# sleepybishop/nanorq

Measured on AMD Instinct MI355X. Metric: Gbit/s encode+decode, K=8192 T=1280, higher is better.
Workload: dtype u8

## Files before the change

__graft_entry__.py:

```python
import os
import sys

ROOT = os.path.dirname(os.path.abspath(__file__))
for p in (ROOT, os.path.join(ROOT, "tests")):
    if p not in sys.path:
        sys.path.insert(0, p)


def build():
    from nanorq_amd import build as nbuild
    nbuild.build_lib(verbose=True)
    nbuild.build_emu()
    nbuild.build_planner_emu()
    nbuild.build_ingest_emu()
    nbuild.build_emit_emu()
    nbuild.build_held_emu()
    nbuild.build_rxset_emu()
    nbuild.build_rxset_lists_emu()
    nbuild.build_rxset_want_emu()
    nbuild.build_txset_emu()
    nbuild.build_syms_emu()
    nbuild.build_syms_set_emu()
    nbuild.build_runs_emu()
    nbuild.build_rxset_runs_emu()
    nbuild.build_obj_emu()
    nbuild.build_shape_emu()
    nbuild.build_launch_emu()
    nbuild.build_out_lists_emu()
    nbuild.build_model_lib()
    nbuild.build_rows_probe()
    nbuild.build_tools()
    import oracle
    oracle.build()
    if os.path.isfile("/root/reference/benchmark.c"):
        import subprocess
        subprocess.run(["make", "-s", "-C", os.path.join(ROOT, "oracle"), "_ref/benchmark_hip", "_ref/encode_hip", "_ref/decode_hip"],
                       check=True)
    import nanorq_amd
    nanorq_amd.lib()
    print("build ok:", nanorq_amd.lib_path())


def smoke():
    import numpy as np
    import nanorq_amd
    import oracle
    import gpu_support as G
    from util import payload, loss_pattern

    K, T, nblk = 1024, 1280, 2
    src = np.stack([payload(K * T, seed=1, block=b).reshape(K, T) for b in range(nblk)])
    lost = [loss_pattern(K, 0.05, seed=2, block=b) for b in range(nblk)]
    nrep = max(len(l) for l in lost) + 2
    esis = np.arange(K, K + nrep, dtype=np.uint32)
    rep, inter = G.gpu_encode(src, K, T, esis, want_inter=True)
    for b in range(nblk):
        r_rep, r_int, _ = oracle.encode_block(src[b], K, T, esis, want_inter=True)
        assert np.array_equal(inter[b], r_int), "intermediate symbols differ from the oracle"
        assert np.array_equal(rep[b], r_rep), "repair symbols differ from the oracle"
    work = src.copy()
    for b in range(nblk):
        work[b][lost[b]] = 0
    st, out, _ = G.gpu_decode(work, K, T, lost, [esis[:len(l) + 2] for l in lost],
                              [rep[b][:len(lost[b]) + 2] for b in range(nblk)])
    assert st.all() and np.array_equal(out, src), "decode mismatch"
    print("smoke ok: K=%d T=%d blocks=%d, stats=%s" % (K, T, nblk, G.ctx().stats()))


if __name__ == "__main__":
    build()
    if "--smoke" in sys.argv:
        smoke()
```

include/nanorq_hip.h:

```cpp
#ifndef NANORQ_HIP_H
#define NANORQ_HIP_H

#include <stddef.h>
#include <stdint.h>

#ifdef __cplusplus
extern "C" {
#endif

typedef struct nrq_ctx nrq_ctx;

typedef struct nrq_call_stats {
  double plan_ms;
  double host_ms;
  uint32_t strip_bytes;
  uint32_t lds_bytes;
  uint32_t grid;
  uint32_t planner;
  uint64_t plan_bytes;
  uint64_t xor_ops;
  uint32_t npiv, u, nlev, nfree;
  uint32_t wg_threads;
  uint32_t strips_per_slot;
  uint32_t wg_waves_per_simd;
  uint32_t host_planned;
  uint32_t movers_aligned;
  uint32_t plan_ahead;
  uint32_t strip_bytes_b, blocks_b;
  uint32_t plan_wg_threads;
  uint32_t plan_compact_state;
  uint32_t plan_segmented;
  uint32_t backsub_strip;
  uint32_t encplan_device;
} nrq_call_stats;

int nrq_ctx_create(int device, void *stream, nrq_ctx **out);
void nrq_ctx_destroy(nrq_ctx *ctx);
int nrq_ctx_set_stream(nrq_ctx *ctx, void *stream);
const char *nrq_ctx_error(nrq_ctx *ctx);
int nrq_ctx_sync(nrq_ctx *ctx);
void nrq_ctx_last_stats(nrq_ctx *ctx, nrq_call_stats *out);
int nrq_ctx_set_planner(nrq_ctx *ctx, int device_planner);
int nrq_ctx_set_option(nrq_ctx *ctx, const char *name, long long value);
int nrq_ctx_set_threads(nrq_ctx *ctx, int n);

int nrq_params(uint32_t K, uint32_t out[10]);

int nrq_precalculate(nrq_ctx *ctx, uint32_t K, uint32_t Kp);
int nrq_warm(nrq_ctx *ctx, uint32_t K, uint32_t Kp, int encode_plan);
void nrq_plan_cache_clear(nrq_ctx *ctx);

int nrq_encode_blocks(nrq_ctx *ctx, uint32_t K, uint32_t Kp, uint32_t T, uint32_t nblk, const void *d_src, size_t src_stride,
                      void *d_inter, size_t inter_stride, uint32_t nrep, const uint32_t *h_esis, void *d_rep,
                      size_t rep_stride);

int nrq_decode_blocks(nrq_ctx *ctx, uint32_t K, uint32_t Kp, uint32_t T, uint32_t nblk, void *d_src, size_t src_stride,
                      const uint32_t *h_lost, const uint32_t *h_nlost, uint32_t lost_cap, const uint32_t *h_rep_esi,
                      const uint32_t *h_nrep, uint32_t rep_cap, const void *d_rep, size_t rep_stride, void *d_inter,
                      size_t inter_stride, int *h_status);

int nrq_decode_blocks_lazy(nrq_ctx *ctx, uint32_t K, uint32_t Kp, uint32_t T, uint32_t nblk, void *d_src, size_t src_stride,
                           const uint32_t *h_lost, const uint32_t *h_nlost, uint32_t lost_cap, const uint32_t *h_rep_esi,
                           const uint32_t *h_nrep, const uint32_t *h_nrep_avail, uint32_t rep_cap, const void *d_rep,
                           size_t rep_stride, void *d_inter, size_t inter_stride, int *h_status, uint32_t *h_used);

int nrq_decode_plan_ahead(nrq_ctx *ctx, uint32_t K, uint32_t Kp, uint32_t T, uint32_t nblk, void *d_src, size_t src_stride,
                          const uint32_t *h_lost, const uint32_t *h_nlost, uint32_t lost_cap, const uint32_t *h_rep_esi,
                          const uint32_t *h_nrep, const uint32_t *h_nrep_avail, uint32_t rep_cap, const void *d_rep, size_t rep_stride,
                          void *d_inter, size_t inter_stride);

int nrq_encode_blocks_v(nrq_ctx *ctx, uint32_t K, uint32_t Kp, uint32_t T, uint32_t nblk, const void *d_src, size_t src_stride,
                        const uint64_t *d_inter_v);
int nrq_decode_blocks_v(nrq_ctx *ctx, uint32_t K, uint32_t Kp, uint32_t T, uint32_t nblk, const uint64_t *d_src_v, const uint32_t *h_lost,
                        const uint32_t *h_nlost, uint32_t lost_cap, const uint32_t *h_rep_esi, const uint32_t *h_nrep,
                        const uint32_t *h_nrep_avail, uint32_t rep_cap, const uint64_t *d_rep_v, int *h_status, uint32_t *h_used);

int nrq_decode_blocks_vi(nrq_ctx *ctx, uint32_t K, uint32_t Kp, uint32_t T, uint32_t nblk, const uint64_t *d_src_v, const uint32_t *h_lost,
                         const uint32_t *h_nlost, uint32_t lost_cap, const uint32_t *h_rep_esi, const uint32_t *h_nrep,
                         const uint32_t *h_nrep_avail, uint32_t rep_cap, const uint64_t *d_rep_v, const uint64_t *d_inter_v, int *h_status,
                         uint32_t *h_used);

int nrq_decode_blocks_vc(nrq_ctx *ctx, uint32_t K, uint32_t Kp, uint32_t T, uint32_t nblk, const uint64_t *d_src_v, const uint32_t *h_lost,
                         const uint32_t *h_nlost, uint32_t lost_cap, const uint32_t *h_rep_esi, const uint32_t *h_nrep,
                         const uint32_t *h_nrep_avail, uint32_t rep_cap, const uint64_t *d_rep_v, int *h_status, uint32_t *h_used,
                         uint32_t chunk_blocks, void *const *chunk_done, void *const *upload_done);

int nrq_gen_symbols(nrq_ctx *ctx, uint32_t K, uint32_t Kp, uint32_t T, uint32_t nblk, const void *d_inter, size_t inter_stride,
                    uint32_t n, const uint32_t *h_isi, void *d_out, size_t out_stride);

int nrq_gen_symbols_dev(nrq_ctx *ctx, uint32_t K, uint32_t Kp, uint32_t T, uint32_t nblk, const void *d_inter, size_t inter_stride,
                        uint32_t n, const uint32_t *d_isi, void *d_out, size_t out_stride);

int nrq_dev_alloc(nrq_ctx *ctx, size_t bytes, void **out);
int nrq_dev_free(nrq_ctx *ctx, void *p);
int nrq_dev_upload(nrq_ctx *ctx, void *d_dst, const void *h_src, size_t bytes);
int nrq_dev_download(nrq_ctx *ctx, void *h_dst, const void *d_src, size_t bytes);
int nrq_dev_memset(nrq_ctx *ctx, void *d_dst, int value, size_t bytes);
int nrq_dev_upload_async(nrq_ctx *ctx, void *d_dst, const void *h_src, size_t bytes);
int nrq_dev_download_async(nrq_ctx *ctx, void *h_dst, const void *d_src, size_t bytes);
int nrq_dev_copy(nrq_ctx *ctx, void *d_dst, const void *d_src, size_t bytes);

int nrq_dev_trim(nrq_ctx *ctx);
int nrq_dev_pool_books(nrq_ctx *ctx, size_t out[3]);

int nrq_host_alloc_pinned(size_t bytes, void **out);
void nrq_host_free_pinned(void *p);
int nrq_host_register(void *p, size_t bytes);
void nrq_host_unregister(void *p);
int nrq_host_is_pinned(const void *p);
int nrq_host_range_is_pinned(const void *p, size_t bytes);
int nrq_copy_on(nrq_ctx *ctx, int stream, void *dst, const void *src, size_t bytes);
int nrq_memset_on(nrq_ctx *ctx, int stream, void *d_dst, int value, size_t bytes);
int nrq_event_new(nrq_ctx *ctx, void **out);
void nrq_event_free(void *ev);
int nrq_event_record(nrq_ctx *ctx, void *ev, int stream);
int nrq_stream_wait(nrq_ctx *ctx, int stream, void *ev);
// ... 154 lines not shown
```

nanorq_amd/binding.py:

```python
import ctypes as C
import os

import numpy as np

_HERE = os.path.dirname(os.path.abspath(__file__))
_LIB = None


class NrqError(RuntimeError):
    pass


class ObjParams(C.Structure):
    _fields_ = [("F", C.c_uint64)] + [(n, C.c_uint32) for n in
                                       ("T", "Al", "Z", "N", "Kt", "ZL", "KL", "KpL", "ZS", "KS", "KpS", "NL", "TL", "NS", "TS",
                                        "flags", "max_esi")] + [("oti_common", C.c_uint64), ("oti_specific", C.c_uint32)]

    def as_dict(self):
        return {n: getattr(self, n) for n, _ in self._fields_}


class CallStats(C.Structure):
    _fields_ = [("plan_ms", C.c_double), ("host_ms", C.c_double), ("strip_bytes", C.c_uint32),
                ("lds_bytes", C.c_uint32), ("grid", C.c_uint32), ("planner", C.c_uint32),
                ("plan_bytes", C.c_uint64), ("xor_ops", C.c_uint64), ("npiv", C.c_uint32), ("u", C.c_uint32),
                ("nlev", C.c_uint32), ("nfree", C.c_uint32), ("wg_threads", C.c_uint32), ("strips_per_slot", C.c_uint32),
                ("wg_waves_per_simd", C.c_uint32), ("host_planned", C.c_uint32), ("movers_aligned", C.c_uint32),
                ("plan_ahead", C.c_uint32), ("strip_bytes_b", C.c_uint32), ("blocks_b", C.c_uint32),
                ("plan_wg_threads", C.c_uint32), ("plan_compact_state", C.c_uint32), ("plan_segmented", C.c_uint32),
                ("backsub_strip", C.c_uint32), ("encplan_device", C.c_uint32)]

    def as_dict(self):
        return {k: getattr(self, k) for k, _ in self._fields_}


def lib_path():
    return os.path.join(_HERE, "libnanorq_hip.so")


def lib():
    global _LIB
    if _LIB is not None:
        return _LIB
    from . import build
    path = os.environ.get("NANORQ_HIP_LIB") or build.build_lib()
    L = C.CDLL(path)
    vp, u32p, ip = C.c_void_p, C.POINTER(C.c_uint32), C.POINTER(C.c_int)
    sz = C.c_size_t
    L.nrq_ctx_create.argtypes = [C.c_int, vp, C.POINTER(vp)]
    L.nrq_ctx_destroy.argtypes = [vp]
    L.nrq_ctx_destroy.restype = None
    L.nrq_ctx_set_stream.argtypes = [vp, vp]
    L.nrq_ctx_error.argtypes = [vp]
    L.nrq_ctx_error.restype = C.c_char_p
    L.nrq_ctx_sync.argtypes = [vp]
    L.nrq_ctx_last_stats.argtypes = [vp, C.POINTER(CallStats)]
    L.nrq_ctx_last_stats.restype = None
    L.nrq_ctx_set_threads.argtypes = [vp, C.c_int]
    L.nrq_ctx_set_planner.argtypes = [vp, C.c_int]
    L.nrq_ctx_set_option.argtypes = [vp, C.c_char_p, C.c_longlong]
    L.nrq_params.argtypes = [C.c_uint32, u32p]
    L.nrq_precalculate.argtypes = [vp, C.c_uint32, C.c_uint32]
    L.nrq_plan_cache_clear.argtypes = [vp]
    L.nrq_plan_cache_clear.restype = None
    L.nrq_encode_blocks.argtypes = [vp, C.c_uint32, C.c_uint32, C.c_uint32, C.c_uint32, vp, sz, vp, sz, C.c_uint32, u32p, vp, sz]
    L.nrq_decode_blocks.argtypes = [vp, C.c_uint32, C.c_uint32, C.c_uint32, C.c_uint32, vp, sz, u32p, u32p, C.c_uint32, u32p,
                                    u32p, C.c_uint32, vp, sz, vp, sz, ip]
    L.nrq_decode_blocks_lazy.argtypes = [vp, C.c_uint32, C.c_uint32, C.c_uint32, C.c_uint32, vp, sz, u32p, u32p, C.c_uint32,
                                         u32p, u32p, u32p, C.c_uint32, vp, sz, vp, sz, ip, u32p]
    L.nrq_decode_plan_ahead.argtypes = [vp, C.c_uint32, C.c_uint32, C.c_uint32, C.c_uint32, vp, sz, u32p, u32p, C.c_uint32,
                                        u32p, u32p, u32p, C.c_uint32, vp, sz, vp, sz]
    L.nrq_gen_symbols.argtypes = [vp, C.c_uint32, C.c_uint32, C.c_uint32, C.c_uint32, vp, sz, C.c_uint32, u32p, vp, sz]
    L.nrq_dev_alloc.argtypes = [vp, sz, C.POINTER(vp)]
    L.nrq_dev_free.argtypes = [vp, vp]
    if hasattr(L, "nrq_dev_pool_books"):
        L.nrq_dev_pool_books.argtypes = [vp, C.POINTER(sz)]
    L.nrq_dev_trim.argtypes = [vp]
    L.nrq_dev_upload.argtypes = [vp, vp, vp, sz]
    L.nrq_dev_download.argtypes = [vp, vp, vp, sz]
    L.nrq_dev_memset.argtypes = [vp, vp, C.c_int, sz]
    L.nrq_ktime_enable.argtypes = [vp, C.c_int]
    L.nrq_ktime_read.argtypes = [vp, C.POINTER(C.c_float), C.c_uint32, u32p]
    L.nrq_ptime_read.argtypes = [vp, C.POINTER(C.c_float), C.c_uint32, u32p]
    L.nrq_ktime_read_intervals.argtypes = [vp, vp, C.POINTER(C.c_float), C.POINTER(C.c_float), C.c_uint32, u32p]
    L.nrq_timer_start.argtypes = [vp]
    L.nrq_timer_stop_ms.argtypes = [vp, C.POINTER(C.c_float)]
    L.nrq_rx_create.argtypes = [vp, C.c_uint32, C.c_uint32, C.c_uint32, C.c_uint32, C.c_uint32, C.c_uint32, C.c_uint32, vp, sz, vp, sz,
                                C.POINTER(vp)]
    L.nrq_rx_destroy.argtypes = [vp]
    L.nrq_rx_destroy.restype = None
    L.nrq_rx_add.argtypes = [vp, vp, sz, vp, C.c_uint32, C.c_uint32, vp]
    L.nrq_rx_counts.argtypes = [vp, u32p, u32p]
    L.nrq_rx_lists.argtypes = [vp, u32p, u32p, u32p, u32p]
    L.nrq_rx_decode.argtypes = [vp, ip, u32p]
    L.nrq_rx_src.argtypes = [vp]
    L.nrq_rx_src.restype = vp
    L.nrq_rx_rep.argtypes = [vp]
    L.nrq_rx_rep.restype = vp
    L.nrq_rx_reset.argtypes = [vp]
    L.nrq_tx_create.argtypes = [vp, C.c_uint32, C.c_uint32, C.c_uint32, C.c_uint32, C.c_uint32, vp, sz, C.POINTER(vp)]
    L.nrq_tx_destroy.argtypes = [vp]
    L.nrq_tx_destroy.restype = None
    L.nrq_tx_encode.argtypes = [vp]
    L.nrq_tx_emit.argtypes = [vp, vp, C.c_uint32, vp, sz, C.c_uint32, vp]
    L.nrq_tx_emit_range.argtypes = [vp, C.c_uint32, C.c_uint32, C.c_int, vp, sz, C.c_uint32, vp]
    L.nrq_tx_inter.argtypes = [vp]
    L.nrq_tx_inter.restype = vp
    opp = C.POINTER(ObjParams)
    L.nrq_obj_params_enc.argtypes = [C.c_uint64, C.c_uint32, C.c_uint32, C.c_uint32, C.c_uint32, C.c_uint32, C.c_uint32, opp]
    L.nrq_obj_params_oti.argtypes = [C.c_uint64, C.c_uint32, C.c_uint32, opp]
    L.nrq_obj_layout.argtypes = [vp, opp, vp, vp, C.c_int]
    L.nrq_otx_create.argtypes = [vp, opp, vp, C.POINTER(vp)]
    L.nrq_otx_destroy.argtypes = [vp]
# ... 3 lines not shown
    L.nrq_otx_emit_all.argtypes = [vp, C.c_uint32, C.c_int, vp, sz, C.c_uint32, vp]
    L.nrq_otx_oti.argtypes = [vp, C.POINTER(C.c_uint64), u32p]
    L.nrq_orx_create.argtypes = [vp, opp, C.c_uint32, C.POINTER(vp)]
    L.nrq_orx_destroy.argtypes = [vp]
    L.nrq_orx_destroy.restype = None
    L.nrq_orx_add.argtypes = [vp, vp, sz, vp, C.c_uint32, C.c_uint32, vp]
    L.nrq_orx_counts.argtypes = [vp, u32p, u32p]
    L.nrq_orx_decode.argtypes = [vp, ip, u32p]
    L.nrq_orx_write.argtypes = [vp, vp]
    if hasattr(L, "nrq_rx_relay"):
        L.nrq_tx_ready.argtypes = [vp, u32p]
        L.nrq_rx_relay.argtypes = [vp, C.POINTER(vp)]
        L.nrq_otx_ready.argtypes = [vp, u32p]
        L.nrq_orx_relay.argtypes = [vp, C.POINTER(vp)]
    if hasattr(L, "nrq_rx_held"):
        L.nrq_rx_held.argtypes = [vp, vp, C.c_uint32, u32p]
        L.nrq_orx_held.argtypes = [vp, vp, C.c_uint32, u32p]
    if hasattr(L, "nrq_rx_want"):
        L.nrq_rx_want.argtypes = [vp, C.c_uint32, C.c_uint32, C.c_uint32, vp, C.c_uint32, u32p]
        L.nrq_orx_want.argtypes = [vp, C.c_uint32, C.c_uint32, C.c_uint32, vp, C.c_uint32, u32p]
    if hasattr(L, "nrq_rxset_create"):
        L.nrq_rxset_create.argtypes = [vp, C.c_uint32, C.POINTER(vp)]
        L.nrq_rxset_destroy.argtypes = [vp]
        L.nrq_rxset_destroy.restype = None
        L.nrq_rxset_attach.argtypes = [vp, C.c_uint32, vp]
        L.nrq_rxset_attach_obj.argtypes = [vp, C.c_uint32, vp]
        L.nrq_rxset_detach.argtypes = [vp, C.c_uint32]
        L.nrq_rxset_add.argtypes = [vp, vp, sz, vp, vp, C.c_uint32, C.c_uint32, vp]
    if hasattr(L, "nrq_rxset_decode"):
        L.nrq_rxset_blocks.argtypes = [vp, u32p, u32p, C.c_uint32, u32p]
        L.nrq_rxset_counts.argtypes = [vp, u32p, u32p]
        L.nrq_rxset_lists.argtypes = [vp, u32p, u32p, u32p, sz, C.POINTER(sz)]
        L.nrq_rxset_decode.argtypes = [vp, ip, u32p]
    if hasattr(L, "nrq_rxset_want"):
        L.nrq_rxset_want.argtypes = [vp, C.c_uint32, C.c_uint32, C.c_uint32, vp, vp, C.c_uint32, u32p, u32p]
        L.nrq_rxset_held.argtypes = [vp, vp, vp, C.c_uint32, u32p, u32p]
    if hasattr(L, "nrq_txset_create"):
        L.nrq_txset_create.argtypes = [vp, C.c_uint32, C.POINTER(vp)]
        L.nrq_txset_destroy.argtypes = [vp]
        L.nrq_txset_destroy.restype = None
        L.nrq_txset_attach.argtypes = [vp, C.c_uint32, vp]
        L.nrq_txset_attach_obj.argtypes = [vp, C.c_uint32, vp]
        L.nrq_txset_detach.argtypes = [vp, C.c_uint32]
        L.nrq_txset_blocks.argtypes = [vp, u32p, u32p, C.c_uint32, u32p]
        L.nrq_txset_emit.argtypes = [vp, vp, vp, C.c_uint32, vp, sz, C.c_uint32, vp]
    if hasattr(L, "nrq_rx_add_syms"):
        u32 = C.c_uint32
        L.nrq_pkt_count.argtypes = [u32, u32, u32, u32]
        L.nrq_pkt_count.restype = u32
        L.nrq_rx_add_syms.argtypes = [vp, vp, sz, vp, u32, u32, vp, u32, vp]
        L.nrq_orx_add_syms.argtypes = [vp, vp, sz, vp, u32, u32, vp, u32, vp]
        L.nrq_tx_emit_syms.argtypes = [vp, vp, u32, u32, vp, vp, sz, u32, vp]
        L.nrq_otx_emit_syms.argtypes = [vp, vp, u32, u32, vp, vp, sz, u32, vp]
        L.nrq_tx_emit_range_syms.argtypes = [vp, u32, u32, u32, C.c_int, vp, sz, u32, vp, vp, u32p]
        L.nrq_otx_emit_all_syms.argtypes = [vp, u32, u32, C.c_int, vp, sz, u32, vp, vp, u32p]
    if hasattr(L, "nrq_rxset_add_syms"):
        u32 = C.c_uint32
        L.nrq_rxset_add_syms.argtypes = [vp, vp, sz, vp, vp, u32, u32, vp, u32, vp]
        L.nrq_txset_emit_syms.argtypes = [vp, vp, vp, u32, u32, vp, vp, sz, u32, vp]
    if hasattr(L, "nrq_rx_want_syms"):
        u32 = C.c_uint32
        L.nrq_rx_want_syms.argtypes = [vp, u32, u32, u32, u32, vp, vp, u32, u32p, u32p]
        L.nrq_orx_want_syms.argtypes = [vp, u32, u32, u32, u32, vp, vp, u32, u32p, u32p]
        L.nrq_rx_held_syms.argtypes = [vp, u32, vp, vp, u32, u32p, u32p]
        L.nrq_orx_held_syms.argtypes = [vp, u32, vp, vp, u32, u32p, u32p]
    if hasattr(L, "nrq_rxset_want_syms"):
        u32 = C.c_uint32
        L.nrq_rxset_want_syms.argtypes = [vp, u32, u32, u32, u32, vp, vp, vp, u32, u32p, u32p, u32p]
        L.nrq_rxset_held_syms.argtypes = [vp, u32, vp, vp, vp, u32, u32p, u32p, u32p]
    u8pp = C.POINTER(C.POINTER(C.c_uint8))
    L.nrq_host_kconst_build.argtypes = [C.c_uint32, u8pp, u32p]
    L.nrq_host_plan_build.argtypes = [C.c_uint32, C.c_uint32, u32p, C.POINTER(C.c_uint8), u8pp, u32p]
    L.nrq_host_plan_build_forced.argtypes = [C.c_uint32, C.c_uint32, u32p, C.POINTER(C.c_uint8), u8pp, u32p, C.c_uint32]
    L.nrq_host_free.argtypes = [vp]
    L.nrq_host_free.restype = None
    _LIB = L
    return L


PARAM_NAMES = ("Kp", "J", "S", "H", "W", "L", "P", "P1", "U", "B")
PLAN_FIELDS = ("magic status K Kp J S H W L P P1 B M npiv u nlow r2 nfree nlev nrows pipe wpr "
               "npiv_pad n_xor_ops off_ops off_pivslot off_pivcol off_wt off_lowslot off_pivx off_fbits "
               "off_mh off_freex off_hinv off_colslot off_pivof off_uslot total_bytes reserved0 reserved1 fail_site "
               "off_augt lpr aug_stride nneed need_pad off_needslot off_wneed").split()


def params(K):
    out = (C.c_uint32 * 10)()
    if lib().nrq_params(K, out) != 0:
        raise ValueError("K out of range: %r" % (K,))
    return dict(zip(PARAM_NAMES, (int(x) for x in out)))


def _u32(a):
    return a.ctypes.data_as(C.POINTER(C.c_uint32))


def host_kconst(K):
    out = C.POINTER(C.c_uint8)()
    n = C.c_uint32()
    if lib().nrq_host_kconst_build(K, C.byref(out), C.byref(n)) != 0:
        raise NrqError("kconst build failed")
    buf = bytes(C.string_at(out, n.value))
    lib().nrq_host_free(out)
    return buf


def host_plan(K, isis, kconst, extra_inact=0):
    isis = np.ascontiguousarray(isis, dtype=np.uint32)
    kc = (C.c_uint8 * len(kconst)).from_buffer_copy(kconst)
    out = C.POINTER(C.c_uint8)()
    n = C.c_uint32()
    rc = lib().nrq_host_plan_build_forced(K, len(isis), _u32(isis), kc, C.byref(out), C.byref(n), int(extra_inact))
    if rc != 0:
        raise NrqError("plan build failed: %d" % rc)
    buf = bytes(C.string_at(out, n.value))
    lib().nrq_host_free(out)
    return buf


def plan_header(plan):
    h = np.frombuffer(plan, dtype=np.uint32, count=len(PLAN_FIELDS))
    return dict(zip(PLAN_FIELDS, (int(x) for x in h)))


class Context:

    def __init__(self, device=0, stream=None):
        self._L = lib()
        h = C.c_void_p()
        rc = self._L.nrq_ctx_create(device, C.c_void_p(stream or 0), C.byref(h))
        if rc != 0:
            raise NrqError("nrq_ctx_create failed (%d): no usable HIP device -- the HIP path has no CPU fallback" % rc)
        self._h = h
        self.device = device

    def close(self):
        if getattr(self, "_h", None):
            self._L.nrq_ctx_destroy(self._h)
            self._h = None

    def __del__(self):
        try:
            self.close()
        except Exception:
            pass

    def _chk(self, rc):
        if rc != 0:
            raise NrqError("%s (rc=%d)" % (self._L.nrq_ctx_error(self._h).decode(), rc))

    def set_stream(self, stream):
        self._chk(self._L.nrq_ctx_set_stream(self._h, C.c_void_p(stream or 0)))

    def set_planner(self, device=True):
        self._chk(self._L.nrq_ctx_set_planner(self._h, int(bool(device))))

    def set_option(self, name, value):
        self._chk(self._L.nrq_ctx_set_option(self._h, name.encode(), int(value)))

    def set_threads(self, n):
        self._chk(self._L.nrq_ctx_set_threads(self._h, n))

    def sync(self):
        self._chk(self._L.nrq_ctx_sync(self._h))

    def stats(self):
# ... 777 lines not shown
```

nanorq_amd/build.py:

```python
import os
import shutil
import subprocess
import sys

HERE = os.path.dirname(os.path.abspath(__file__))
ROOT = os.path.dirname(HERE)
CSRC = os.path.join(HERE, "csrc")
LIB = os.path.join(HERE, "libnanorq_hip.so")
EMU = os.path.join(ROOT, "tests", "emu", "libsolve_emu.so")
PEMU = os.path.join(ROOT, "tests", "emu", "libplanner_emu.so")
IEMU = os.path.join(ROOT, "tests", "emu", "libingest_emu.so")
XEMU = os.path.join(ROOT, "tests", "emu", "libemit_emu.so")
OEMU = os.path.join(ROOT, "tests", "emu", "libobj_emu.so")
SEMU = os.path.join(ROOT, "tests", "emu", "libshape_emu.so")
HEMU = os.path.join(ROOT, "tests", "emu", "libheld_emu.so")
WEMU = os.path.join(ROOT, "tests", "emu", "libwant_emu.so")
REMU = os.path.join(ROOT, "tests", "emu", "librxset_emu.so")
LEMU = os.path.join(ROOT, "tests", "emu", "librxset_lists_emu.so")
QEMU = os.path.join(ROOT, "tests", "emu", "librxset_want_emu.so")
TEMU = os.path.join(ROOT, "tests", "emu", "libtxset_emu.so")
YEMU = os.path.join(ROOT, "tests", "emu", "libsyms_emu.so")
ZEMU = os.path.join(ROOT, "tests", "emu", "libsyms_set_emu.so")
GEMU = os.path.join(ROOT, "tests", "emu", "libruns_emu.so")
JEMU = os.path.join(ROOT, "tests", "emu", "librxset_runs_emu.so")
NEMU = os.path.join(ROOT, "tests", "emu", "liblaunch_emu.so")
UEMU = os.path.join(ROOT, "tests", "emu", "libout_lists_emu.so")
MODEL = os.path.join(ROOT, "tests", "emu", "libnanorq_model.so")
ROWS = os.path.join(ROOT, "tests", "gpu", "librows_probe.so")

HIP_SOURCES = ["nrq_device.hip"]
CXX_SOURCES = ["planner_host.cpp"]
C_SOURCES = ["nanorq_api.c", "io.c"]


def _hipcc():
    for c in (os.environ.get("HIPCC"), "/opt/rocm/bin/hipcc", shutil.which("hipcc")):
        if c and os.path.exists(c):
            return c
    raise RuntimeError("hipcc not found: the HIP extension cannot be built (no CPU fallback exists)")


def _newer(target, deps):
    if not os.path.exists(target):
        return True
    t = os.path.getmtime(target)
    return any(os.path.getmtime(d) > t for d in deps if os.path.exists(d))


def _deps():
    out = []
    for d in (CSRC, os.path.join(ROOT, "include")):
        for f in os.listdir(d):
            out.append(os.path.join(d, f))
    return out


def build_lib(force=False, verbose=False, out=None, extra=(), host_extra=(), reuse_hip_obj=False):
    if out is None and not force and not _newer(LIB, _deps()):
        return LIB
    hipcc = _hipcc()
    objdir = os.path.join(HERE, "build" if out is None else "build_" + os.path.basename(out))
    os.makedirs(objdir, exist_ok=True)
    objs = []
    common = ["-O3", "-fPIC", "-Wno-pass-failed", "-I" + os.path.join(ROOT, "include"), "-I" + CSRC]
    common += list(extra)
    headers = [f for f in _deps() if f.endswith(".h")]

    def stale(o, src):
        return force or out is not None or _newer(o, [src] + headers)

    for s in HIP_SOURCES:
        o = os.path.join(objdir, s + ".o")
        if reuse_hip_obj and os.path.exists(os.path.join(HERE, "build", s + ".o")):
            objs.append(os.path.join(HERE, "build", s + ".o"))
            continue
        if stale(o, os.path.join(CSRC, s)):
            subprocess.run([hipcc, "--offload-arch=gfx950", "-std=c++17", *common, "-c", os.path.join(CSRC, s), "-o", o],
                           check=True)
        objs.append(o)
    for s in CXX_SOURCES:
        o = os.path.join(objdir, s + ".o")
        if stale(o, os.path.join(CSRC, s)):
            subprocess.run(["g++", "-std=c++17", "-Wall", *common, *host_extra, "-c", os.path.join(CSRC, s), "-o", o], check=True)
        objs.append(o)
    for s in C_SOURCES:
        src = os.path.join(CSRC, s)
        if not os.path.exists(src):
            continue
        o = os.path.join(objdir, s + ".o")
        if stale(o, src):
            subprocess.run(["gcc", "-std=gnu11", "-Wall", "-D_FILE_OFFSET_BITS=64", *common, *host_extra, "-c", src, "-o", o], check=True)
        objs.append(o)
    target = out or LIB
    subprocess.run([hipcc, "--offload-arch=gfx950", "-shared", "-fPIC", "-o", target, *objs, "-lpthread"], check=True)
    if verbose:
        print("built", target)
    return target


def build_tools(force=False):
    src = os.path.join(ROOT, "tools", "rqfile.c")
    exe = os.path.join(ROOT, "tools", "rqfile")
    deps = [src, LIB] + [os.path.join(ROOT, "include", h) for h in ("nanorq.h", "nanorq_batch.h", "io.h")]
    if force or _newer(exe, deps):
        subprocess.run(["gcc", "-std=c99", "-D_DEFAULT_SOURCE", "-D_FILE_OFFSET_BITS=64", "-O2", "-Wall", "-I" + os.path.join(ROOT, "include"),
                        src, "-o", exe, "-L" + os.path.dirname(LIB), "-lnanorq_hip", "-Wl,-rpath,$ORIGIN/../nanorq_amd", "-lm"], check=True)
    return exe


def _build_emu(target, src, headers, force):
    if force or _newer(target, [src] + [os.path.join(CSRC, h) for h in headers]):
        subprocess.run(["g++", "-O2", "-std=c++17", "-Wall", "-Wno-unknown-pragmas", "-fPIC", "-shared", "-o", target, src], check=True)
    return target


def build_emu(force=False):
    return _build_emu(EMU, os.path.join(ROOT, "tests", "emu", "solve_emu.cpp"),
                      ("solve_body.h", "split_body.h", "plan.h", "rq_math.h", os.path.join(ROOT, "tests", "emu", "strip_emu.h")), force)


def build_launch_emu(force=False):
    return _build_emu(NEMU, os.path.join(ROOT, "tests", "emu", "launch_emu.cpp"),
                      ("launch_shape.h", "planner_body.h", "solve_body.h", "split_body.h", "plan.h", "rq_math.h", "rfc6330_tables.h",
                       os.path.join(ROOT, "tests", "emu", "strip_emu.h"), os.path.join(ROOT, "tests", "emu", "wave_emu.h")), force)


def build_planner_emu(force=False):
    return _build_emu(PEMU, os.path.join(ROOT, "tests", "emu", "planner_emu.cpp"),
                      ("planner_body.h", "planner_seq.h", "solve_body.h", "plan.h", "rq_math.h"), force)


def build_out_lists_emu(force=False):
    return _build_emu(UEMU, os.path.join(ROOT, "tests", "emu", "out_lists_emu.cpp"), ("out_lists.h", "rq_math.h"), force)


def build_ingest_emu(force=False):
    return _build_emu(IEMU, os.path.join(ROOT, "tests", "emu", "ingest_emu.cpp"), ("ingest_body.h",), force)


def build_emit_emu(force=False):
    return _build_emu(XEMU, os.path.join(CSRC, "emit_emu.cpp"), ("emit_emu.h", "emit_body.h", "rq_math.h"), force)


def build_held_emu(force=False):
    return _build_emu(HEMU, os.path.join(CSRC, "held_emu.cpp"), ("emit_emu.h", "emit_body.h", "held_body.h", "ingest_body.h", "rq_math.h"), force)


def build_want_emu(force=False):
    return _build_emu(WEMU, os.path.join(CSRC, "want_emu.cpp"), ("want_body.h", "held_body.h", "ingest_body.h"), force)


def build_rxset_emu(force=False):
    return _build_emu(REMU, os.path.join(CSRC, "rxset_emu.cpp"), ("ingest_set_body.h", "ingest_body.h"), force)


def build_rxset_lists_emu(force=False):
    return _build_emu(LEMU, os.path.join(CSRC, "rxset_lists_emu.cpp"),
                      ("lists_set_body.h", "rxset_plan.h", "ingest_set_body.h", "ingest_body.h"), force)


def build_rxset_want_emu(force=False):
    return _build_emu(QEMU, os.path.join(CSRC, "rxset_want_emu.cpp"),
                      ("emu_scan.h", "want_set_body.h", "lists_set_body.h", "want_body.h", "held_body.h", "ingest_set_body.h", "ingest_body.h"), force)


def build_txset_emu(force=False):
    return _build_emu(TEMU, os.path.join(CSRC, "txset_emu.cpp"), ("emit_set_body.h", "emit_body.h", "rq_math.h"), force)


def build_syms_emu(force=False):
    return _build_emu(YEMU, os.path.join(CSRC, "syms_emu.cpp"), ("emit_emu.h", "syms_body.h", "emit_body.h", "ingest_body.h", "rq_math.h"), force)


def build_syms_set_emu(force=False):
    return _build_emu(ZEMU, os.path.join(CSRC, "syms_set_emu.cpp"),
                      ("syms_set_body.h", "syms_body.h", "ingest_set_body.h", "emit_set_body.h", "emit_body.h", "ingest_body.h", "rq_math.h"), force)


def build_runs_emu(force=False):
    return _build_emu(GEMU, os.path.join(CSRC, "runs_emu.cpp"),
                      ("emit_emu.h", "runs_emu_walks.h", "runs_body.h", "syms_body.h", "want_body.h", "held_body.h", "emit_body.h", "ingest_body.h",
                       "rq_math.h"), force)


def build_rxset_runs_emu(force=False):
    return _build_emu(JEMU, os.path.join(CSRC, "rxset_runs_emu.cpp"),
                      ("emu_scan.h", "runs_emu_walks.h", "runs_set_body.h", "runs_body.h", "syms_set_body.h", "want_set_body.h", "lists_set_body.h",
                       "syms_body.h", "want_body.h", "held_body.h", "emit_set_body.h", "emit_body.h", "ingest_set_body.h", "ingest_body.h", "rq_math.h"), force)


def build_obj_emu(force=False):
    return _build_emu(OEMU, os.path.join(ROOT, "tests", "emu", "obj_emu.cpp"), ("obj_body.h", "emit_body.h", "rq_math.h"), force)


def build_shape_emu(force=False):
    return _build_emu(SEMU, os.path.join(ROOT, "tests", "emu", "shape_emu.cpp"),
                      ("launch_shape.h", "planner_body.h", "solve_body.h", "plan.h", "rq_math.h", "rfc6330_tables.h"), force)


def build_model_lib(force=False, out=None, sanitize=False):
    emu = os.path.join(ROOT, "tests", "emu")
    hook, model, effects = os.path.join(emu, "hip_model.h"), os.path.join(emu, "hip_model.cpp"), os.path.join(emu, "model_effects.cpp")
    target = out or MODEL
    if not force and not _newer(target, _deps() + [hook, model, effects]):
        return target
    hipcc = _hipcc()
    rocm = os.path.dirname(os.path.dirname(os.path.realpath(hipcc)))
    objdir = os.path.join(HERE, "build_model" if out is None else "build_" + os.path.basename(out))
    os.makedirs(objdir, exist_ok=True)
    common = ["-O2", "-g1", "-fPIC", "-I" + os.path.join(ROOT, "include"), "-I" + CSRC, "-I" + emu]
    cc, cxx, san, hip_san = "gcc", "g++", [], []
    if sanitize:
        llvm = os.path.join(rocm, "lib", "llvm", "bin")
        cc, cxx = os.path.join(llvm, "clang"), os.path.join(llvm, "clang++")
        san = ["-O1", "-fno-omit-frame-pointer", "-fsanitize=address,undefined", "-fno-sanitize-recover=undefined"]
        hip_san = [x for f in san for x in ("-Xarch_host", f)]
    objs = []

    def obj(cmd, src, name):
        o = os.path.join(objdir, name + ".o")
        subprocess.run([*cmd, *common, "-c", src, "-o", o], check=True)
        objs.append(o)
        return o

    dev = obj([hipcc, "--offload-host-only", "-std=c++17", "-Wno-pass-failed", "-DNRQ_HIP_MODEL_HOOK", "-include", hook, *hip_san],
              os.path.join(CSRC, HIP_SOURCES[0]), HIP_SOURCES[0])
    for s in CXX_SOURCES:
        obj([cxx, "-std=c++17", "-Wall", *san], os.path.join(CSRC, s), s)
    for s in C_SOURCES:
        obj([cc, "-std=gnu11", "-Wall", "-D_FILE_OFFSET_BITS=64", *san], os.path.join(CSRC, s), s)
    obj([cxx, "-std=c++17", "-Wall", "-D__HIP_PLATFORM_AMD__", "-I" + os.path.join(rocm, "include"), *san], model, "hip_model.cpp")
    obj([cxx, "-std=c++17", "-Wall", "-Wno-unknown-pragmas", *[f for f in san if f != "-fsanitize=address,undefined"],
         *(["-fsanitize=undefined"] if sanitize else [])], effects, "model_effects.cpp")
    undefined = subprocess.run(["nm", "-u", dev], check=True, stdout=subprocess.PIPE).stdout.decode().split()
    defs = ["-Wl,--defsym=%s=0" % n for n in undefined if n.startswith("__hip_fatbin")]
    subprocess.run([cxx, "-shared", "-fPIC", *san, "-o", target, *objs, *defs, "-lpthread", "-ldl"], check=True)
    return target


def build_rows_probe(force=False):
    src = os.path.join(ROOT, "tests", "gpu", "rows_probe.hip")
    if force or _newer(ROWS, [src, os.path.join(CSRC, "solve_body.h"), os.path.join(CSRC, "plan.h")]):
        subprocess.run([_hipcc(), "--offload-arch=gfx950", "-O3", "-std=c++17", "-I" + CSRC, "-shared", "-fPIC", src, "-o", ROWS], check=True)
    return ROWS


def build_model_exercise(force=False, sanitize=True):
    emu = os.path.join(ROOT, "tests", "emu")
    src = os.path.join(emu, "model_exercise.cpp")
    exe = os.path.join(emu, "model_exercise_asan" if sanitize else "model_exercise")
    lib = build_model_lib(force=force, out=os.path.join(emu, "libnanorq_model_asan.so") if sanitize else None, sanitize=sanitize)
    if force or _newer(exe, [src, lib]):
        cxx, san = "g++", []
        if sanitize:
            cxx = os.path.join(os.path.dirname(os.path.dirname(os.path.realpath(_hipcc()))), "lib", "llvm", "bin", "clang++")
            san = ["-O1", "-fno-omit-frame-pointer", "-fsanitize=address,undefined", "-fno-sanitize-recover=undefined"]
        subprocess.run([cxx, "-std=c++17", "-Wall", "-g1", *san, "-I" + os.path.join(ROOT, "include"), "-I" + emu, src, "-o", exe,
                        "-L" + emu, "-l:" + os.path.basename(lib), "-Wl,-rpath,$ORIGIN", "-lpthread"], check=True)
    return exe


if __name__ == "__main__":
    build_lib(force="-f" in sys.argv, verbose=True)
    build_emu(force="-f" in sys.argv)
    build_planner_emu(force="-f" in sys.argv)
    build_ingest_emu(force="-f" in sys.argv)
    build_emit_emu(force="-f" in sys.argv)
    build_held_emu(force="-f" in sys.argv)
    build_want_emu(force="-f" in sys.argv)
    build_rxset_emu(force="-f" in sys.argv)
    build_rxset_lists_emu(force="-f" in sys.argv)
    build_rxset_want_emu(force="-f" in sys.argv)
    build_txset_emu(force="-f" in sys.argv)
    build_syms_emu(force="-f" in sys.argv)
    build_syms_set_emu(force="-f" in sys.argv)
    build_runs_emu(force="-f" in sys.argv)
    build_rxset_runs_emu(force="-f" in sys.argv)
    build_obj_emu(force="-f" in sys.argv)
    build_shape_emu(force="-f" in sys.argv)
    build_launch_emu(force="-f" in sys.argv)
    build_out_lists_emu(force="-f" in sys.argv)
    build_model_lib(force="-f" in sys.argv)
    build_rows_probe(force="-f" in sys.argv)
    build_tools(force="-f" in sys.argv)
```

nanorq_amd/csrc/nrq_device.hip:

```cpp
#include <hip/hip_runtime.h>

#include <algorithm>
#include <atomic>
#include <chrono>
#include <cstdarg>
#include <cstdio>
#include <cstdlib>
#include <cstring>
#include <deque>
#include <map>
#include <new>
#include <string>
#include <thread>
#include <vector>

#include "../../include/nanorq_hip.h"
#include "plan.h"
#include "planner_host.h"
#include "rq_math.h"
#include "out_lists.h"
#include "solve_body.h"
#include "split_body.h"
#include "planner_body.h"
#include "ingest_body.h"
// ... 351 lines not shown
  pl_tag_pl_scan_b = 0,
  pl_tag_pl_scan_c = 0,
  pl_tag_pl_pcsc_fill = 0,
#endif
  pl_tag_pl_round_claim = 1,
  pl_tag_pl_round_drop = 3,
  pl_tag_pl_round_chain_end = 3,
  pl_tag_pl_inact_find = 5,
  pl_tag_pl_inact_find_b = 5,
  pl_tag_pl_inact_find_c = 5,
  pl_tag_pl_inact_apply_a = 6,
  pl_tag_pl_inact_apply_b = 6,
  pl_tag_pl_inact_next = 6,
  pl_tag_pl_event_scan = 5,
  pl_tag_pl_event_pick = 6,
  pl_tag_pl_event_drop = 6,
  pl_tag_pl_lev_0 = 7,
  pl_tag_pl_pivot_sort = 7,
  pl_tag_pl_lev_a = 7,
  pl_tag_pl_check_a = 7,
  pl_tag_pl_check_b = 7,
  pl_tag_pl_check_c = 7,
  pl_tag_pl_lev_b = 7,
  pl_tag_pl_w_init = 8,
  pl_tag_pl_w_init_b = 8,
  pl_tag_pl_cls_fetch = 8,
  pl_tag_pl_w_group = 8,
  pl_tag_pl_w_stage = 8,
  pl_tag_pl_wfast_spill = 4,
  pl_tag_pl_wfast_load = 4,
  pl_tag_pl_wfast_store = 4,
  pl_tag_pl_wfast_restore = 4,
  pl_tag_pl_low_a = 9,
  pl_tag_pl_low_b = 9,
  pl_tag_pl_low_c = 9,
  pl_tag_pl_ops_layout_a = 10,
  pl_tag_pl_ops_layout = 10,
  pl_tag_pl_ops_clear = 10,
  pl_tag_pl_ops_emit = 10,
  pl_tag_pl_ops_check_a = 10,
  pl_tag_pl_ops_check_b = 10,
  pl_tag_pl_ops_check_c = 10,
  pl_tag_pl_sh_restore = 0,
  pl_tag_pl_sh_save = 15,
  pl_tag_pl_mh_ext_clear = 15,
  pl_tag_pl_mh_fetch = 11,
  pl_tag_pl_mh_init = 11,
  pl_tag_pl_mh_load = 11,
  pl_tag_pl_mh_acc = 11,
  pl_tag_pl_gj_a = 12,
  pl_tag_pl_gjp_init = 12,
  pl_tag_pl_gjp_bid = 12,
  pl_tag_pl_gjp_step = 12,
  pl_tag_pl_gjp_wave = 12,
  pl_tag_pl_mhrev_load = 11,
  pl_tag_pl_mhrev_load_b = 11,
  pl_tag_pl_mhrev_store = 11,
  pl_tag_pl_mhrev_scatter = 11,
  pl_tag_pl_gjp_comb = 12,
  pl_tag_pl_gjp_stage = 12,
  pl_tag_pl_gjp_apply = 12,
  pl_tag_pl_gj_b = 12,
  pl_tag_pl_bin_a = 13,
  pl_tag_pl_bin_b = 13,
  pl_tag_pl_bin_c = 13,
  pl_tag_pl_dense_a = 14,
  pl_tag_pl_dense_b = 14,
  pl_tag_pl_dense_step_a = 14,
  pl_tag_pl_dense_step_b = 14,
  pl_tag_pl_dense_c = 14,
  pl_tag_pl_extra_a = 14,
  pl_tag_pl_extra_b = 14,
  pl_tag_pl_extra_c = 14,
  pl_tag_pl_extra_d = 14,
  pl_tag_pl_final_a = 15,
  pl_tag_pl_final_b = 15,
  pl_tag_pl_final_c = 15,
  pl_tag_pl_final_c2 = 15,
  pl_tag_pl_final_c3 = 15,
  pl_tag_pl_final_d = 15,
  pl_tag_pl_final_e = 15,
  pl_tag_pl_need_a = 15,
  pl_tag_pl_need_b = 15,
  pl_tag_pl_mark_failed = 15,
};

template <int NT, int PK = 0>
__global__ __launch_bounds__(NT) __attribute__((amdgpu_waves_per_eu(NT <= 256 ? 5 : 1)))
void nrq_plan_kernel(rq_params p, const uint8_t *__restrict__ kc,
                                                         const nrq_planjob *__restrict__ pjobs,
                                                         nrq_job *__restrict__ jobs_out, uint32_t nblk, uint32_t Mcap,
                                                         uint32_t npcap, uint32_t ucap, uint32_t lds_dyn_bytes,
                                                         unsigned long long *__restrict__ prof, uint32_t seg, uint32_t qcap,
                                                         uint32_t lowcap) {
  extern __shared__ __attribute__((aligned(16))) uint8_t smem[];
  const uint32_t b = blockIdx.x, tid = threadIdx.x;
#define PL_SEG_ (PK == 0 ? 0u : seg)
  if (b >= nblk) return;
  uint8_t *dyn = smem;
  pl_shared *sh = reinterpret_cast<pl_shared *>(smem + lds_dyn_bytes);
  PlanCtx c;
  pl_ctx_setup(c, p, kc, pjobs[b], sh, dyn, lds_dyn_bytes, Mcap, npcap, ucap, jobs_out + b, qcap, lowcap, (uint32_t)NT);
  if (!PK) c.pk_cnt = c.pk_un = c.pk_pa = c.pk_vb = nullptr;
  if (PL_SEG_ == 3u) c.cls_glob = reinterpret_cast<uint32_t *>(c.work + c.wl.cls_g);
  unsigned long long t_prev = prof ? (unsigned long long)clock64() : 0ull;
#ifdef PL_STAMP
#define PL_ACC(tag) ((void)0)
#else
#define PL_ACC(tag) do { if (__builtin_expect(prof && b == 0 && tid == 0, 0)) { unsigned long long t_ = (unsigned long long)clock64(); \
                                                          prof[tag] += t_ - t_prev; prof[16 + tag] += 1; t_prev = t_; } } while (0)
#endif
#define PL_PHASE(fn) do { fn<PK>(c, tid, (uint32_t)NT); __syncthreads(); PL_ACC(pl_tag_##fn); } while (0)
#define PL_PHASE1(fn, a) do { fn<PK>(c, (a), tid, (uint32_t)NT); __syncthreads(); PL_ACC(pl_tag_##fn); } while (0)
#ifndef PL_CLAIM_FULL_BARRIER
#define PL_CLAIM_FULL_BARRIER 0
#endif
#ifndef PL_CLAIM_SKIP_IDLE
#define PL_CLAIM_SKIP_IDLE 1
#endif
#define PL_PHASE1_CLAIM(fn, a) do { if (!PL_CLAIM_SKIP_IDLE || (tid & ~63u) < nq_) fn<PK>(c, (a), tid, (uint32_t)NT); \
    if (!PL_CLAIM_FULL_BARRIER && (pl_peel_in_lds(c) || c.pk_cnt)) asm volatile("s_waitcnt lgkmcnt(0)\n\ts_barrier" ::: "memory"); else __syncthreads(); \
    PL_ACC(pl_tag_##fn); } while (0)
#define PL_WFAST_RUN(wb) do { \
    if (tid < NRQ_ROW) { \
      const NRQ_GAS uint32_t *ops_ = gptr<uint32_t>(c.arena + c.sh->off_ops); \
      if ((wb) == 16u) fwd_rows<16>(ops_, pl_wfast_rows(c), tid); \
      else if ((wb) == 8u) fwd_rows<8>(ops_, pl_wfast_rows(c), tid); \
      else fwd_rows<4>(ops_, pl_wfast_rows(c), tid); \
    } \
    __syncthreads(); PL_ACC(2); } while (0)
#define PL_MHREV_RUN(wb) do { \
    if (tid < NRQ_ROW) { \
      const NRQ_GAS uint32_t *ops_ = gptr<uint32_t>(c.arena + c.sh->off_ops); \
      if ((wb) == 16u) rev_rows<16>(ops_, pl_wfast_rows(c), tid); \
      else if ((wb) == 8u) rev_rows<8>(ops_, pl_wfast_rows(c), tid); \
      else rev_rows<4>(ops_, pl_wfast_rows(c), tid); \
    } \
    __syncthreads(); PL_ACC(11); } while (0)
#define PL_SEG PL_SEG_
#define PL_STEER_SYNC __syncthreads()
#define PL_NT_ ((uint32_t)NT)
#define PL_Z ((uint32_t)PK)
#ifdef PL_STAMP
  c.st_on = prof && b == 0 && tid == 0; c.st_prev = 0; c.st_blk = prof && b == 0;
  if (tid < 32) sh->st_acc[tid] = 0;
  __syncthreads();
#endif
  if (PL_SEG_ == 2u || PL_SEG_ == 4u) PL_PHASE(pl_sh_restore);
#include "planner_seq.h"
#ifdef PL_STAMP
  if (c.st_on) { for (int i_ = 0; i_ < 32; i_++) prof[32 + i_] = sh->st_acc[i_]; }
#endif
  if (PL_SEG_ == 1u || PL_SEG_ == 4u) PL_PHASE(pl_mh_ext_clear);
  if (PL_SEG_ == 1u || PL_SEG_ == 3u || PL_SEG_ == 4u) PL_PHASE(pl_sh_save);
#undef PL_SEG
#undef PL_SEG_
#undef PL_STEER_SYNC
#undef PL_NT_
#undef PL_PHASE
#undef PL_PHASE1
#undef PL_PHASE1_CLAIM
#undef PL_WFAST_RUN
#undef PL_MHREV_RUN
#undef PL_Z
#undef PL_ACC
}
// ... 904 lines not shown
  if (rc) return rc;
  memset(&ctx->stats, 0, sizeof(ctx->stats));
  ctx->stats.plan_ms = cached ? 0.0 : ep->build_ms;
  ctx->stats.plan_bytes = ep->plan_bytes;
  ctx->stats.xor_ops = (uint64_t)ep->hdr.n_xor_ops * nblk;
  ctx->stats.npiv = ep->hdr.npiv; ctx->stats.u = ep->hdr.u; ctx->stats.nlev = ep->hdr.nlev;
  ctx->stats.nfree = ep->hdr.nfree;
  ctx->stats.encplan_device = ep->dev_built ? 1u : 0u;

  std::vector<uint32_t> isis(nrep), cptr, order;
  std::vector<uint16_t> cols;
  for (uint32_t q = 0; q < nrep; q++) isis[q] = h_esis[q] + (p.Kp - K);
  build_out_lists(p, ep->colslot.data(), nrep, isis.data(), cptr, cols, order);
  const size_t off_jobs = 0;
  const size_t off_cptr = r16(off_jobs + (size_t)nblk * sizeof(nrq_job));
  const size_t off_row = r16(off_cptr + (size_t)(nrep + 1) * 4);
  const size_t off_cols = r16(off_row + (size_t)(nrep ? nrep : 1) * 4);
  const size_t total = r16(off_cols + cols.size() * 2 + NRQ_STORE_SLACK);
  const int f = ctx->flip;
  ctx->flip ^= 1;
  HIPCHK(ctx, hipEventSynchronize(ctx->staged[f]));
  if ((rc = ensure_pin(ctx, ctx->staging[f], total))) return rc;
  if ((rc = ensure_dev(ctx, ctx->scratch[f], total))) return rc;
  uint8_t *hs = ctx->staging[f].p, *ds = ctx->scratch[f].p;
  memcpy(hs + off_cptr, cptr.data(), (size_t)(nrep + 1) * 4);
  if (nrep) memcpy(hs + off_row, order.data(), (size_t)nrep * 4);
  if (!cols.empty()) memcpy(hs + off_cols, cols.data(), cols.size() * 2);
  nrq_job *jobs = reinterpret_cast<nrq_job *>(hs + off_jobs);
  for (uint32_t b = 0; b < nblk; b++) {
    nrq_job &j = jobs[b];
    memset(&j, 0, sizeof(j));
    j.plan = (uint64_t)(uintptr_t)ep->dev;
    j.rowsrc = (uint64_t)(uintptr_t)(ep->dev + ep->rowsrc_off);
    j.src = src.of(b);
    j.rep = 0;
    j.inter = inter ? inter.of(b) : 0;
    j.out = nrep ? rep.of(b) : 0;
    j.out_cptr = (uint64_t)(uintptr_t)(ds + off_cptr);
    j.out_slots = (uint64_t)(uintptr_t)(ds + off_cols);
    j.out_row = (uint64_t)(uintptr_t)(ds + off_row);
    j.nout = nrep;
  }
  HIPCHK(ctx, hipMemcpyAsync(ds, hs, total, hipMemcpyHostToDevice, ctx->stream));
  HIPCHK(ctx, hipEventRecord(ctx->staged[f], ctx->stream));
  std::vector<const nrq_plan_hdr *> hdrs(1, &ep->hdr);
  rc = pick_and_launch(ctx, hdrs, reinterpret_cast<const nrq_job *>(ds + off_jobs), nblk, T, kc->dev.p, (inter ? p.L : 0u) + nrep, io_aligned);
  if (ep->used[ep->cur]) {
    HIPCHK(ctx, hipEventRecord(ep->used[ep->cur], ctx->stream));
    ep->used_set[ep->cur] = true;
  }
  ctx->stats.host_ms = now_ms() - t_begin;
  return rc;
}

int nrq_encode_blocks(nrq_ctx *ctx, uint32_t K, uint32_t Kp, uint32_t T, uint32_t nblk, const void *d_src, size_t src_stride,
                      void *d_inter, size_t inter_stride, uint32_t nrep, const uint32_t *h_esis, void *d_rep,
                      size_t rep_stride) {
  if (!ctx) return -1;
  return encode_blocks(ctx, K, Kp, T, nblk, Rows{d_src, src_stride}, Rows{d_inter, inter_stride}, nrep, h_esis, Rows{d_rep, rep_stride});
}

int nrq_encode_blocks_v(nrq_ctx *ctx, uint32_t K, uint32_t Kp, uint32_t T, uint32_t nblk, const void *d_src, size_t src_stride,
                        const uint64_t *d_inter_v) {
  if (!ctx || !d_inter_v) return -1;
  return encode_blocks(ctx, K, Kp, T, nblk, Rows{d_src, src_stride}, Rows{nullptr, 0, d_inter_v}, 0, nullptr, Rows{});
}

static int decode_host(nrq_ctx *ctx, const DecodeCall &c, const uint8_t *select) {
  const uint32_t K = c.K, T = c.T, nblk = c.nblk;
  const double t_begin = now_ms();
  rq_params p;
  int rc = block_params(ctx, K, c.Kp, &p);
  if (rc) return rc;
  KConst *kc;
  rc = get_kconst(ctx, p.Kp, &kc);
  if (rc) return rc;
  if (!select) memset(&ctx->stats, 0, sizeof(ctx->stats));

  struct Prep {
    HostBuf plan;
    uint32_t plan_bytes = 0;
    std::vector<uint32_t> rowsrc, cptr, orow;
    std::vector<uint16_t> cols;
    int state = 0;
    uint32_t used = 0;
    size_t off_plan = 0, off_rowsrc = 0, off_cptr = 0, off_row = 0, off_cols = 0;
  };
  std::vector<Prep> prep(nblk);
  const uint32_t pad = p.Kp - K;

  auto prepare = [&](uint32_t b) {
    Prep &pr = prep[b];
    const uint32_t nl = c.h_nlost[b], nr = c.h_nrep[b];
    if (select && !select[b]) { pr.state = 2; return; }
    if (nl == 0) { pr.state = 0; return; }
    if (nr < nl || nl > c.lost_cap || nr > c.rep_cap) { pr.state = -1; return; }
    const uint32_t *lost = c.h_lost + (size_t)b * c.lost_cap;
    const uint32_t *resi = c.h_rep_esi + (size_t)b * c.rep_cap;
    uint32_t avail = c.h_avail ? c.h_avail[b] : nr;
    if (avail < nr) avail = nr;
    if (avail > c.rep_cap) avail = c.rep_cap;
    for (uint32_t use = nr;; use++) {
      const uint32_t overhead = use - nl;
      const uint32_t M = p.L + overhead;
      if (M > 65535u) { pr.state = -1; return; }
      std::vector<uint32_t> isis(p.Kp + overhead);
      for (uint32_t j = 0; j < p.Kp; j++) isis[j] = j;
      pr.rowsrc.assign(M, NRQ_ROW_ZERO);
      for (uint32_t j = 0; j < K; j++) pr.rowsrc[p.S + p.H + j] = j;
      for (uint32_t g = 0; g < nl; g++) {
        if (lost[g] >= K || (g && lost[g] <= lost[g - 1]) || resi[g] < K || resi[g] >= (1u << 24)) { pr.state = -1; return; }
        isis[lost[g]] = resi[g] + pad;
        pr.rowsrc[p.S + p.H + lost[g]] = NRQ_ROW_REP | g;
      }
      for (uint32_t e = 0; e < overhead; e++) {
        if (resi[nl + e] < K || resi[nl + e] >= (1u << 24)) { pr.state = -1; return; }
        isis[p.Kp + e] = resi[nl + e] + pad;
        pr.rowsrc[p.L + e] = NRQ_ROW_REP | (nl + e);
      }
      pr.plan = HostBuf();
      if (nrq_host_plan_build_forced(p.Kp, p.Kp + overhead, isis.data(), kc->host.p, &pr.plan.p, &pr.plan_bytes, ctx->tune.plan_force_inact) != 0) {
        pr.state = -1;
        return;
      }
      if (reinterpret_cast<const nrq_plan_hdr *>(pr.plan.p)->status == 0) { pr.used = use; break; }
      if (use + 1 > avail) { pr.state = -1; return; }
    }
    build_out_lists(p, reinterpret_cast<const uint16_t *>(pr.plan.p + reinterpret_cast<const nrq_plan_hdr *>(pr.plan.p)->off_colslot),
                    nl, lost, pr.cptr, pr.cols, pr.orow);
    for (uint32_t &g : pr.orow) g = lost[g];
    pr.state = 1;
  };

  const double t_plan0 = now_ms();
  {
    uint32_t nth = ctx->threads > 0 ? (uint32_t)ctx->threads : std::thread::hardware_concurrency();
    if (nth == 0) nth = 1;
    if (nth > nblk) nth = nblk;
    if ((uint64_t)K * nblk < 920u) nth = 1;
    std::atomic<uint32_t> next(0);
    auto worker = [&]() {
      for (;;) {
        uint32_t b = next.fetch_add(1);
        if (b >= nblk) break;
        prepare(b);
      }
    };
    if (nth <= 1) worker();
    else {
      std::vector<std::thread> pool;
      for (uint32_t t = 0; t < nth; t++) pool.emplace_back(worker);
      for (auto &t : pool) t.join();
    }
  }
  ctx->stats.plan_ms += now_ms() - t_plan0;

  size_t off = r16((size_t)nblk * sizeof(nrq_job));
  const size_t off_dummy = off;
  off = r16(off + sizeof(nrq_plan_hdr));
  uint32_t nsolve = 0;
  for (uint32_t b = 0; b < nblk; b++) {
    Prep &pr = prep[b];
    if (pr.state != 2) { c.h_status[b] = pr.state >= 0 ? 1 : 0; if (c.h_used) c.h_used[b] = pr.state == 1 ? pr.used : 0; }
    if (pr.state != 1) continue;
    nsolve++;
    pr.off_plan = off;   off = r16(off + pr.plan_bytes);
    pr.off_rowsrc = off; off = r16(off + pr.rowsrc.size() * 4);
    pr.off_cptr = off;   off = r16(off + pr.cptr.size() * 4);
    pr.off_row = off;    off = r16(off + pr.orow.size() * 4);
    pr.off_cols = off;   off = r16(off + pr.cols.size() * 2 + NRQ_STORE_SLACK);
  }
  const size_t total = off;
  int result = 0;
  if (nsolve) {
    const int f = ctx->flip;
    ctx->flip ^= 1;
    HIPCHK(ctx, hipEventSynchronize(ctx->staged[f]));
    if ((rc = ensure_pin(ctx, ctx->staging[f], total))) return rc;
    if ((rc = ensure_dev(ctx, ctx->scratch[f], total))) return rc;
    uint8_t *hs = ctx->staging[f].p, *ds = ctx->scratch[f].p;
    nrq_plan_hdr dummy;
    memset(&dummy, 0, sizeof(dummy));
    dummy.magic = NRQ_PLAN_MAGIC;
    dummy.status = 1;
    memcpy(hs + off_dummy, &dummy, sizeof(dummy));
    nrq_job *jobs = reinterpret_cast<nrq_job *>(hs);
    std::vector<const nrq_plan_hdr *> hdrs;
    std::vector<uint32_t> hblk;
    for (uint32_t b = 0; b < nblk; b++) {
      Prep &pr = prep[b];
      nrq_job &j = jobs[b];
      memset(&j, 0, sizeof(j));
      if (pr.state != 1) { j.plan = (uint64_t)(uintptr_t)(ds + off_dummy); continue; }
      hblk.push_back(b);
      memcpy(hs + pr.off_plan, pr.plan.p, pr.plan_bytes);
      memcpy(hs + pr.off_rowsrc, pr.rowsrc.data(), pr.rowsrc.size() * 4);
      memcpy(hs + pr.off_cptr, pr.cptr.data(), pr.cptr.size() * 4);
      memcpy(hs + pr.off_row, pr.orow.data(), pr.orow.size() * 4);
      if (!pr.cols.empty()) memcpy(hs + pr.off_cols, pr.cols.data(), pr.cols.size() * 2);
      const nrq_plan_hdr *h = reinterpret_cast<const nrq_plan_hdr *>(hs + pr.off_plan);
      hdrs.push_back(h);
      if (ctx->stats.npiv == 0) {
        ctx->stats.npiv = h->npiv; ctx->stats.u = h->u; ctx->stats.nlev = h->nlev; ctx->stats.nfree = h->nfree;
      }
      ctx->stats.xor_ops += h->n_xor_ops;
      ctx->stats.plan_bytes += pr.plan_bytes;
      j.plan = (uint64_t)(uintptr_t)(ds + pr.off_plan);
      j.rowsrc = (uint64_t)(uintptr_t)(ds + pr.off_rowsrc);
      j.src = c.src_of(b);
      j.rep = c.rep_of(b);
      j.inter = c.inter_of(b);
      j.out = j.src;
      j.out_cptr = (uint64_t)(uintptr_t)(ds + pr.off_cptr);
      j.out_slots = (uint64_t)(uintptr_t)(ds + pr.off_cols);
      j.out_row = (uint64_t)(uintptr_t)(ds + pr.off_row);
      j.nout = (uint32_t)pr.orow.size();
    }
    hipError_t e = hipMemcpyAsync(ds, hs, total, hipMemcpyHostToDevice, ctx->stream);
    if (e == hipSuccess) e = hipEventRecord(ctx->staged[f], ctx->stream);
    if (e != hipSuccess) result = fail(ctx, -10, "staging copy failed: %s", hipGetErrorString(e));
    else {
      uint32_t max_out = 0;
      for (uint32_t b = 0; b < nblk; b++)
        if (prep[b].state == 1 && prep[b].orow.size() > max_out) max_out = (uint32_t)prep[b].orow.size();
      result = pick_and_launch(ctx, hdrs, reinterpret_cast<const nrq_job *>(ds), nblk, T, kc->dev.p, (c.inter ? p.L : 0u) + max_out, c.io_aligned, &hblk);
    }
  }
  ctx->stats.host_ms += now_ms() - t_begin;
  return result;
}


struct PlanRun {
  rq_params p;
  KConst *kc = nullptr;
  uint32_t ucap = 0, Mcap = 0, npcap = 0, arena_cap = 0, max_nl = 0;
  size_t off_hdrs = 0;
  int f = 0, ab = 0;
  hipStream_t ps = nullptr;
  double t_begin = 0;
  DecodeCall call;
  std::vector<uint32_t> lost, nlost, resi, nrep, avail;
  PlanShape shape;
};

static void plan_ahead_drop(nrq_ctx *ctx) {
  for (PlanRun *r : ctx->ahead) {
    (void)hipEventSynchronize(ctx->planned[r->ab]);
    delete r;
  }
  ctx->ahead.clear();
  ctx->ahead_hint = 0;
}

static int plan_launch(nrq_ctx *ctx, PlanRun &r, const DecodeCall &c) {
  const uint32_t K = c.K, nblk = c.nblk;
  r.t_begin = now_ms();
  rq_params &p = r.p;
  int rc = block_params(ctx, K, c.Kp, &p);
  if (rc) return rc;
  KConst *kc;
  rc = get_kconst(ctx, p.Kp, &kc);
  if (rc) return rc;
  r.kc = kc;
  const nrq_kconst_hdr *kh = reinterpret_cast<const nrq_kconst_hdr *>(kc->host.p);
  uint32_t max_oh = 0, max_nrep = 0, max_nl = 0;
  for (uint32_t b = 0; b < nblk; b++) {
    const uint32_t nl = c.h_nlost[b];
    uint32_t nr = c.h_nrep[b];
    if (nl == 0 || nr < nl || nl > c.lost_cap || nr > c.rep_cap) continue;
    if (c.h_avail && c.h_avail[b] > nr) nr = c.h_avail[b] < c.rep_cap ? c.h_avail[b] : c.rep_cap;
    if (nr - nl > max_oh) max_oh = nr - nl;
    if (nr > max_nrep) max_nrep = nr;
    if (nl > max_nl) max_nl = nl;
  }
  r.max_nl = max_nl;
  uint32_t ucap = p.P + 768u;
  if (ucap > 1280u) ucap = 1280u;
  if (ctx->tune.plan_ucap && ctx->tune.plan_ucap < ucap) ucap = ctx->tune.plan_ucap;
  if (ucap < p.P + 32u) return fail(ctx, -5, "K'=%u has too many permanently inactive columns for the device planner", p.Kp);
  const uint32_t Mcap = p.L + max_oh + PL_EXTRA_ROWS + 8u, npcap = max_nrep + PL_EXTRA_ROWS + 8u;
  const pl_work_layout wl = pl_work_plan(p.L, Mcap, npcap, ucap, kh->nnz + npcap * PL_PATCH_STRIDE);
  const uint32_t arena_cap = pl_arena_bound(p.L, Mcap, ucap, kh->nnz + npcap * PL_PATCH_STRIDE, max_nl + 8u);
// ... 85 lines not shown
    for (int k = 0; k < 16; k++) tot += hp[k];
    fprintf(stderr, "[NRQ_PROF] planner nblk=%u total=%llu clk:", nblk, tot);
    for (int k = 0; k < 16; k++) fprintf(stderr, " %s=%llu(%llu)", nm[k], hp[k], hp[16 + k]);
    fprintf(stderr, "\n");
#ifdef PL_STAMP
    fprintf(stderr, "[NRQ_PROF] round stamps (clocks up to point i, summed over the rounds):");
    for (int k = 0; k < 24; k++) fprintf(stderr, " %d:%llu", k, hp[32 + k]);
    fprintf(stderr, "\n[NRQ_PROF] chained peel: entries %llu, group clocks busy %llu (waiting for the rows %llu), claims %llu, phases %llu clocks %llu; flags trip %llu, subtraction trip %llu, claims %llu\n",
            hp[56], hp[57], hp[58], hp[59], hp[61], hp[60], hp[62], hp[63], hp[54]);
#endif
  }
  HIPCHK(ctx, hipMemcpyAsync(hs + off_hdrs, ds + off_hdrs, (size_t)nblk * sizeof(nrq_plan_hdr), hipMemcpyDeviceToHost, ps));
  HIPCHK(ctx, hipEventRecord(ctx->pstaged[f], ps));
  HIPCHK(ctx, hipEventRecord(ctx->planned[ab], ps));
  return 0;
}

static bool plan_run_matches(const PlanRun &r, const DecodeCall &c) {
  const DecodeCall &a = r.call;
  if (c.src.vec || c.rep.vec || c.chunk_blocks) return false;
  if (a.K != c.K || a.Kp != c.Kp || a.T != c.T || a.nblk != c.nblk || a.lost_cap != c.lost_cap || a.rep_cap != c.rep_cap) return false;
  if (!(a.src == c.src) || !(a.rep == c.rep) || !(a.inter == c.inter) || (a.h_avail != nullptr) != (c.h_avail != nullptr)) return false;
  return memcmp(a.h_nlost, c.h_nlost, (size_t)c.nblk * 4) == 0 && memcmp(a.h_nrep, c.h_nrep, (size_t)c.nblk * 4) == 0 &&
         (!c.h_avail || memcmp(a.h_avail, c.h_avail, (size_t)c.nblk * 4) == 0) &&
         memcmp(a.h_lost, c.h_lost, (size_t)c.nblk * c.lost_cap * 4) == 0 &&
         memcmp(a.h_rep_esi, c.h_rep_esi, (size_t)c.nblk * c.rep_cap * 4) == 0;
}

static int decode_device(nrq_ctx *ctx, const DecodeCall &c, std::vector<uint8_t> *fallback) {
  const uint32_t K = c.K, T = c.T, nblk = c.nblk;
  const double t_begin = now_ms();
  memset(&ctx->stats, 0, sizeof(ctx->stats));
  ctx->stats.planner = 1;
  PlanRun local, *run = &local;
  bool ahead = false;
  while (!ctx->ahead.empty()) {
    PlanRun *f = ctx->ahead.front();
    ctx->ahead.pop_front();
    if (plan_run_matches(*f, c)) {
      run = f;
      ahead = true;
      break;
    }
    (void)hipEventSynchronize(ctx->planned[f->ab]);
    delete f;
    if (ctx->ahead.empty()) ctx->ahead_hint = 0;
  }
  struct Owner { PlanRun *r; ~Owner() { delete r; } } owner{ahead ? run : nullptr};
  if (!ahead) {
    const int rc0 = plan_launch(ctx, *run, c);
    if (rc0) return rc0;
  }
  const rq_params &p = run->p;
  KConst *kc = run->kc;
  const int ab = run->ab;
  const uint32_t max_nl = run->max_nl;
  hipStream_t ps = run->ps;
  uint8_t *hs = ctx->pstaging[run->f].p;
  const size_t off_hdrs = run->off_hdrs;
  HIPCHK(ctx, hipEventSynchronize(ctx->planned[ab]));
  ctx->stats.plan_ms = now_ms() - t_begin;
  ctx->stats.plan_ahead = ahead ? 1 : 0;
  ctx->stats.plan_wg_threads = run->shape.wg_threads;
  ctx->stats.plan_compact_state = run->shape.compact;
  ctx->stats.plan_segmented = run->shape.segmented;
  const nrq_plan_hdr *hd = reinterpret_cast<const nrq_plan_hdr *>(hs + off_hdrs);
  std::vector<const nrq_plan_hdr *> hdrs;
  std::vector<uint32_t> hblk;
  bool need_fallback = false;
  for (uint32_t b = 0; b < nblk; b++) {
    if (c.h_used) c.h_used[b] = 0;
    if (c.h_nlost[b] == 0) { c.h_status[b] = 1; continue; }
    if (hd[b].magic != NRQ_PLAN_MAGIC) return fail(ctx, -11, "device planner produced no header for block %u", b);
    if (hd[b].status == 0) {
      c.h_status[b] = 1;
      if (c.h_used) c.h_used[b] = c.h_nrep[b] + hd[b].reserved[1];
      hdrs.push_back(&hd[b]);
      hblk.push_back(b);
      if (ctx->stats.npiv == 0) {
        ctx->stats.npiv = hd[b].npiv; ctx->stats.u = hd[b].u; ctx->stats.nlev = hd[b].nlev; ctx->stats.nfree = hd[b].nfree;
      }
      ctx->stats.xor_ops += hd[b].n_xor_ops;
      ctx->stats.plan_bytes += hd[b].total_bytes;
    } else if (hd[b].reserved[0] == PL_FAIL_CAPACITY) {
      if (ctx->tune.prof || ctx->tune.diag) fprintf(stderr, "[NRQ_PROF] block %u: device planner capacity exceeded at planner_body.h:%u (npiv %u u %u nlev %u nrows %u M %u nlost %u)\n", b, hd[b].fail_site, hd[b].npiv, hd[b].u, hd[b].nlev, hd[b].nrows, hd[b].M, c.h_nlost[b]);
      (*fallback)[b] = 1;
      need_fallback = true;
      c.h_status[b] = 0;
    } else {
      if (ctx->tune.prof || ctx->tune.diag)
        fprintf(stderr, "[NRQ_PROF] block %u: not decodable: status %u reason %u site %u npiv %u u %u nlev %u nlow %u r2 %u nfree %u taken %u\n", b, hd[b].status,
                hd[b].reserved[0], hd[b].fail_site, hd[b].npiv, hd[b].u, hd[b].nlev, hd[b].nlow, hd[b].r2, hd[b].nfree, hd[b].reserved[1]);
      c.h_status[b] = 0;
    }
  }
  int result = 0;
  if (c.chunk_blocks) {
    if (ps != ctx->stream) HIPCHK(ctx, hipStreamWaitEvent(ctx->stream, ctx->planned[ab], 0));
    const uint32_t cb = c.chunk_blocks;
    for (uint32_t c0 = 0, ci = 0; c0 < nblk && !result; c0 += cb, ci++) {
      const uint32_t m = nblk - c0 < cb ? nblk - c0 : cb;
      std::vector<const nrq_plan_hdr *> hc;
      std::vector<uint32_t> hcb;
      for (uint32_t b = c0; b < c0 + m; b++)
        if (c.h_nlost[b] != 0 && hd[b].magic == NRQ_PLAN_MAGIC && hd[b].status == 0) { hc.push_back(&hd[b]); hcb.push_back(b - c0); }
      if (c.chunk_up && c.chunk_up[ci]) HIPCHK(ctx, hipStreamWaitEvent(ctx->stream, (hipEvent_t)c.chunk_up[ci], 0));
      if (!hc.empty())
        result = pick_and_launch(ctx, hc, reinterpret_cast<const nrq_job *>(ctx->plan_jobs[ab].p) + c0, m, T, kc->dev.p, (c.inter ? p.L : 0u) + max_nl, c.io_aligned, &hcb);
      if (c.chunk_done && c.chunk_done[ci]) HIPCHK(ctx, hipEventRecord((hipEvent_t)c.chunk_done[ci], ctx->stream));
    }
    HIPCHK(ctx, hipEventRecord(ctx->arena_free[ab], ctx->stream));
    ctx->arena_busy[ab] = true;
  } else if (!hdrs.empty()) {
    if (ps != ctx->stream) HIPCHK(ctx, hipStreamWaitEvent(ctx->stream, ctx->planned[ab], 0));
    result = pick_and_launch(ctx, hdrs, reinterpret_cast<const nrq_job *>(ctx->plan_jobs[ab].p), nblk, T, kc->dev.p,
                             (c.inter ? p.L : 0u) + max_nl, c.io_aligned, &hblk);
    HIPCHK(ctx, hipEventRecord(ctx->arena_free[ab], ctx->stream));
    ctx->arena_busy[ab] = true;
  }
  ctx->stats.host_ms = now_ms() - t_begin;
  if (result) return result;
  return need_fallback ? 1 : 0;
}

int nrq_decode_plan_ahead(nrq_ctx *ctx, uint32_t K, uint32_t Kp, uint32_t T, uint32_t nblk, void *d_src, size_t src_stride,
                          const uint32_t *h_lost, const uint32_t *h_nlost, uint32_t lost_cap, const uint32_t *h_rep_esi,
                          const uint32_t *h_nrep, const uint32_t *h_nrep_avail, uint32_t rep_cap, const void *d_rep, size_t rep_stride,
                          void *d_inter, size_t inter_stride) {
  if (!ctx) return -1;
  if (!d_src || T == 0 || nblk == 0 || !h_nlost || !h_nrep || !h_lost || !h_rep_esi) return fail(ctx, -1, "bad arguments");
  if (!ctx->planner) return 0;
  HIPCHK(ctx, hipSetDevice(ctx->device));
  if (ctx->ahead.size() >= NRQ_PLAN_AHEAD_MAX) return fail(ctx, -6, "nrq_decode_plan_ahead: %u runs are already waiting for their decode calls", (unsigned)NRQ_PLAN_AHEAD_MAX);
  DecodeCall c;
  c.K = K; c.Kp = Kp; c.T = T; c.nblk = nblk;
  c.src = {d_src, src_stride}; c.rep = {d_rep, rep_stride}; c.inter = {d_inter, inter_stride};
  c.h_lost = h_lost; c.h_nlost = h_nlost; c.lost_cap = lost_cap;
  c.h_rep_esi = h_rep_esi; c.h_nrep = h_nrep; c.h_avail = h_nrep_avail; c.rep_cap = rep_cap;
  PlanRun *r = new PlanRun();
  const int rc = plan_launch(ctx, *r, c);
  if (rc) { delete r; return rc; }
  r->lost.assign(h_lost, h_lost + (size_t)nblk * lost_cap);
  r->resi.assign(h_rep_esi, h_rep_esi + (size_t)nblk * rep_cap);
  r->nlost.assign(h_nlost, h_nlost + nblk);
  r->nrep.assign(h_nrep, h_nrep + nblk);
  if (h_nrep_avail) r->avail.assign(h_nrep_avail, h_nrep_avail + nblk);
  r->call = c;
  r->call.h_lost = r->lost.data(); r->call.h_nlost = r->nlost.data(); r->call.h_rep_esi = r->resi.data(); r->call.h_nrep = r->nrep.data();
  if (h_nrep_avail) r->call.h_avail = r->avail.data();
  ctx->ahead.push_back(r);
  if (ctx->ahead.size() > ctx->ahead_hint) ctx->ahead_hint = (uint32_t)ctx->ahead.size();
  return 0;
}

static int decode(nrq_ctx *ctx, DecodeCall &c) {
  if (!c.src || c.T == 0 || c.nblk == 0 || !c.h_nlost || !c.h_nrep || !c.h_status) return fail(ctx, -1, "bad arguments");
  HIPCHK(ctx, hipSetDevice(ctx->device));
  const uint32_t K = c.K, nblk = c.nblk;
  c.io_aligned = c.src.aligned(nblk, c.T) && c.rep.aligned(nblk, c.T) && (!c.inter || c.inter.aligned(nblk, c.T));
  const bool host_small = ctx->planner && ctx->tune.host_plan_auto && ctx->ahead.empty() && !c.chunk_blocks &&
                          (uint64_t)38u * nblk * K < (uint64_t)20000u + (uint64_t)28u * K;
  if (!ctx->planner || host_small) {
    const int rc_ = decode_host(ctx, c, nullptr);
    if (host_small) ctx->stats.host_planned = 0;
    return rc_;
  }
// ... 3824 lines not shown
```

nanorq_amd/csrc/out_lists.h:

```cpp
#ifndef NRQ_OUT_LISTS_H
#define NRQ_OUT_LISTS_H
#include <stdint.h>
#include <string.h>
#include <vector>
#include "rq_math.h"

inline void build_out_lists(const rq_params &p, const uint16_t *colslot, uint32_t n, const uint32_t *isis,
                     std::vector<uint32_t> &cptr, std::vector<uint16_t> &cols, std::vector<uint32_t> &order) {
  std::vector<uint32_t> at(n + 1);
  std::vector<uint16_t> byq;
  byq.reserve((size_t)n * 9);
  uint32_t tmp[RQ_MAX_LT_COLS], start[RQ_MAX_LT_COLS + 2] = {0};
  for (uint32_t q = 0; q < n; q++) {
    at[q] = (uint32_t)byq.size();
    const uint32_t m = rq_lt_columns(&p, isis[q], tmp);
    for (uint32_t k = 0; k < m; k++) byq.push_back(colslot[tmp[k]]);
    start[RQ_MAX_LT_COLS - m + 1]++;
  }
  at[n] = (uint32_t)byq.size();
  for (uint32_t l = 0; l <= RQ_MAX_LT_COLS; l++) start[l + 1] += start[l];
  order.resize(n);
  for (uint32_t q = 0; q < n; q++) order[start[RQ_MAX_LT_COLS - (at[q + 1] - at[q])]++] = q;
  cptr.resize(n + 1);
  cols.resize(byq.size());
  uint32_t o = 0;
  for (uint32_t i = 0; i < n; i++) {
    const uint32_t q = order[i], m = at[q + 1] - at[q];
    cptr[i] = o;
    if (m) memcpy(&cols[o], &byq[at[q]], (size_t)m * 2);
    o += m;
  }
  cptr[n] = o;
}

#endif
```

nanorq_amd/csrc/plan.h:

```cpp
#ifndef NRQ_PLAN_H
#define NRQ_PLAN_H

#include <stdint.h>

#define NRQ_PLAN_MAGIC 0x4e525131u
#define NRQ_ROW 64u
#ifndef NRQ_PIPE
#define NRQ_PIPE 2u
#endif
#ifndef NRQ_RING_MULT
#define NRQ_RING_MULT 5u
#endif
#define NRQ_RING (NRQ_RING_MULT * 4u * (NRQ_PIPE + 1u))
#define NRQ_RING_MAX (2u * NRQ_RING)
#define NRQ_PAD_ROWS (2u * NRQ_RING_MAX + NRQ_PIPE + 4u)
#define NRQ_OP_INDEX(row, lane) ((((size_t)(row) >> 2) * NRQ_ROW + (size_t)(lane)) * 4u + ((size_t)(row) & 3u))
#define NRQ_OP_LANE_OF_INDEX(i) ((uint32_t)((i) >> 2) & (NRQ_ROW - 1u))
#define NRQ_STREAM_ROWS(rows) (((rows) + 3u) & ~3u)
#define NRQ_SCRATCH 64u
#define NRQ_OP(dst, src) (((uint32_t)(dst) + NRQ_SCRATCH) | (((uint32_t)(src) + NRQ_SCRATCH) << 16))
#define NRQ_NOP_AT(pos) (((uint32_t)(pos) & (NRQ_ROW - 1u)) * 0x10001u)
#define NRQ_OP_IS_NOP(op) (((op) & 0xFFFFu) < NRQ_SCRATCH)
#define NRQ_OP_DST(op) (((op) & 0xFFFFu) - NRQ_SCRATCH)
#define NRQ_OP_SRC(op) (((op) >> 16) - NRQ_SCRATCH)
#define NRQ_NOSLOT 0xFFFFu
#define NRQ_MAX_FREE 32u

#define NRQ_LANE_CLASSES 8u
#if defined(__HIPCC__)
#define NRQ_PLAN_FN __host__ __device__ static inline
#else
#define NRQ_PLAN_FN static inline
#endif
NRQ_PLAN_FN uint32_t nrq_op_class(uint32_t op) { return op & (NRQ_LANE_CLASSES - 1u); }
NRQ_PLAN_FN uint32_t nrq_group_span(uint32_t n, const uint32_t *cf) {
  uint32_t mf = 0;
  for (uint32_t d = 0; d < NRQ_LANE_CLASSES; d++) mf = cf[d] > mf ? cf[d] : mf;
  const uint32_t need = (mf + NRQ_LANE_CLASSES - 1u) / NRQ_LANE_CLASSES + (NRQ_PIPE - 1u);
  const uint32_t have = (n + NRQ_ROW - 1u) / NRQ_ROW;
  return have > need ? have : need;
}
NRQ_PLAN_FN uint32_t nrq_lane_place(uint32_t span, const uint32_t *ct, uint32_t d, uint32_t r) {
  const uint32_t cap = span * NRQ_LANE_CLASSES;
  if (r >= cap) {
    uint32_t o = r - cap;
    for (uint32_t e = 0; e < d; e++) o += ct[e] > cap ? ct[e] - cap : 0u;
    for (uint32_t e = 0; e < NRQ_LANE_CLASSES; e++) {
      const uint32_t holes = ct[e] < cap ? cap - ct[e] : 0u;
      if (o < holes) { d = e; r = ct[e] + o; break; }
      o -= holes;
    }
  }
  return (r >> 1) * 16u + 2u * d + (r & 1u);
}
#ifndef NRQ_EARLY_NARROW
#define NRQ_EARLY_NARROW 128u
#endif
#ifndef NRQ_MULTI_INACT
#define NRQ_MULTI_INACT 8u
#endif

#ifndef NRQ_AUG_MATRIX_MIN_L
#define NRQ_AUG_MATRIX_MIN_L 5000u
#endif
typedef struct nrq_plan_hdr {
  uint32_t magic;
  uint32_t status;
  uint32_t K, Kp, J, S, H, W, L, P, P1, B;
  uint32_t M;
  uint32_t npiv;
  uint32_t u;
  uint32_t nlow;
  uint32_t r2;
  uint32_t nfree;
  uint32_t nlev;
  uint32_t nrows;
  uint32_t pipe;
  uint32_t wpr;
  uint32_t npiv_pad;
  uint32_t n_xor_ops;

  uint32_t off_ops;
  uint32_t off_pivslot;
  uint32_t off_pivcol;
  uint32_t off_wt;
  uint32_t off_lowslot;
  uint32_t off_pivx;
  uint32_t off_fbits;
  uint32_t off_mh;
  uint32_t off_freex;
  uint32_t off_hinv;
  uint32_t off_colslot;
  uint32_t off_pivof;
  uint32_t off_uslot;
  uint32_t total_bytes;
  uint32_t reserved[2];
  uint32_t fail_site;
  uint32_t off_augt;
  uint32_t lpr;
  uint32_t aug_stride;
  uint32_t nneed;
  uint32_t need_pad;
  uint32_t off_needslot;
  uint32_t off_wneed;
} nrq_plan_hdr;
#ifdef __cplusplus
static_assert(sizeof(nrq_plan_hdr) <= 256u, "nrq_plan_hdr is read as a 256-byte prefix");
#endif

#define NRQ_CHEAD 16u
typedef struct nrq_kconst_hdr {
  uint32_t Kp, S, H, n;
  uint32_t off_g;
  uint32_t off_b12;
  uint32_t total_bytes;
  uint32_t L, W, P, nnz;
  uint32_t off_rptr;
  uint32_t off_cidx;
  uint32_t off_cptr;
  uint32_t off_ridx;
  uint32_t off_state;
  uint32_t off_gt;
  uint32_t off_erow;
  uint32_t off_chead;
} nrq_kconst_hdr;

#endif
```

nanorq_amd/csrc/planner_body.h:

```cpp
#ifndef NRQ_PLANNER_BODY_H
#define NRQ_PLANNER_BODY_H

#include <stdint.h>
#include <string.h>

#include "plan.h"
#include "rq_math.h"
#include "solve_body.h"

#ifndef PL_NT
#define PL_NT 1024u
#endif
#define PL_NT_MIN 256u
#ifndef PL_NT_TINY
#define PL_NT_TINY 128u
#endif
#define PL_QCAP 2048u
#define PL_UNASSIGNED 0x80000000u
#define PL_PATCHED 0x40000000u
#define PL_LEVEL_MASK 0x3FFFFFFFu
#define PL_ST_V 0u
#define PL_ST_PIVOT 1u
#define PL_ST_INACT 2u
#define PL_ST_CLAIM 3u
// ... 142 lines not shown
  uint32_t nV, npiv, ninact, nlev;
  uint32_t nq[2], nclaim[2];
  uint32_t ncand[2];
  uint32_t best;
  uint32_t nlow, r2, nfree, cand[3];
  uint32_t arena_top, nrows, nrec, opbase;
  uint32_t uslot_fill, tmp0, tmp1;
  uint32_t off_ops;
  uint32_t lv_in_lds, opq_group[2];
  uint32_t tmp_mhoff;
  uint32_t dense_ok, nextra, spare_base, spare_fill, xcol, xrow[48];
  uint32_t ndone;
  uint32_t own_hits;
  uint32_t chk_piv, chk_inact;
  uint32_t bkt_n[PL_EMIT_TILES_MAX];
  uint32_t ev_n, ev_min, ev_none;
  uint32_t off_augt, aug_stride, mhrev;
  uint32_t bin_ct[NRQ_LANE_CLASSES];
  uint32_t gj_A[32];
  uint16_t gj_pr[32];
  uint32_t freex[NRQ_MAX_FREE];
  uint8_t gf_exp[512], gf_log[256];
  uint8_t aug[PL_MAXH * (NRQ_MAX_FREE + PL_MAXH)];
  uint8_t solver[NRQ_MAX_FREE];
  uint8_t taken[PL_MAXH];
  uint8_t colf[PL_MAXH];
} pl_shared;
SB_HD uint32_t pl_shared_bytes(uint32_t qcap, uint32_t lowcap, uint32_t nt) {
  return pl_r16((uint32_t)sizeof(pl_shared)) + pl_r16(qcap * 8u) + pl_r16(nt * 4u) + pl_r16(lowcap * 2u);
}

SB_HD bool pl_bin_in_stream(uint32_t L) { return L < NRQ_AUG_MATRIX_MIN_L; }

typedef struct pl_work_layout {
  uint32_t rowstate, rowinfo, colinfo, patch_of, patch_cols, patch_len, pc_ptr, pc_fill, pc_rows, pc_head, ucol, wrows,
      lev_ops, lev_base, lev_fill, pivdeg, lowdeg, lev_fin, red_row, red_x, rec_word, rec_idx, rec_g, cand, sh_save, mh_ext, cls_g, wentry, emit_bkt, chk, total;
} pl_work_layout;

SB_HD pl_work_layout pl_work_plan(uint32_t L, uint32_t Mcap, uint32_t npcap, uint32_t ucap, uint32_t nnzcap) {
  pl_work_layout w;
  uint32_t o = 0;
  const uint32_t wprcap = (ucap + 31u) / 32u;
  w.rowstate = o;   o = pl_r16(o + Mcap * 4u);
  w.rowinfo = o;    o = pl_r16(o + Mcap * 4u);
  w.colinfo = o;    o = pl_r16(o + L * 4u);
  w.patch_of = o;   o = pl_r16(o + Mcap * 2u);
  w.patch_cols = o; o = pl_r16(o + npcap * PL_PATCH_STRIDE * 2u);
  w.patch_len = o;  o = pl_r16(o + npcap);
  w.pc_ptr = o;     o = pl_r16(o + (L + 1u) * 4u);
  w.pc_fill = o;    o = pl_r16(o + (L + 1u) * 4u);
  w.pc_rows = o;    o = pl_r16(o + npcap * PL_PATCH_STRIDE * 2u);
  w.pc_head = o;    o = pl_r16(o + L * PL_PCHEAD * 2u);
  w.ucol = o;       o = pl_r16(o + ucap * 2u);
  w.wrows = o;      o = pl_r16(o + Mcap * wprcap * 4u);
  w.lev_ops = o;    o = pl_r16(o + (L + 2u) * 4u);
  w.lev_base = o;   o = pl_r16(o + (L + 2u) * 4u);
  w.lev_fill = o;   o = pl_r16(o + (L + 2u) * 4u);
  w.pivdeg = o;     o = pl_r16(o + L * 4u);
  w.lowdeg = o;     o = pl_r16(o + Mcap * 4u);
  w.lev_fin = o;    o = pl_r16(o + (L + 2u) * 4u);
  w.red_row = o;    o = pl_r16(o + ucap * 4u);
  w.red_x = o;      o = pl_r16(o + ucap * 4u);
  w.rec_word = o;   o = pl_r16(o + nnzcap * 4u);
  w.rec_idx = o;    o = pl_r16(o + nnzcap * 4u);
  w.rec_g = o;      o = pl_r16(o + nnzcap * 2u);
  w.cand = o;       o = pl_r16(o + Mcap * 2u);
  w.sh_save = o;    o = pl_r16(o + pl_shared_bytes(PL_QCAP, PL_LOWCAP, PL_NT));
  w.mh_ext = o;     o = pl_r16(o + ucap * PL_MAXH);
  w.cls_g = o;      o = pl_r16(o + (L + 2u) * 32u);
  w.wentry = o;     o = pl_r16(o + 16u);
  w.emit_bkt = o;   o = pl_r16(o + 3u * nnzcap * 8u);
  w.chk = o;        o = pl_r16(o + Mcap * 2u);
  w.total = o;
  return w;
}

SB_HD uint32_t pl_arena_bound(uint32_t L, uint32_t Mcap, uint32_t ucap, uint32_t nnz, uint32_t nlost_cap) {
  const uint32_t wprcap = (ucap + 31u) / 32u, npad = (L + 63u) & ~63u;
  uint32_t ops = (2u * nnz + nnz / 2u) + NRQ_ROW * (NRQ_PIPE * (L / 2u + 8u) + PL_SPARE_ROWS + NRQ_PAD_ROWS + 4u);
  if (pl_bin_in_stream(L)) ops += 2u * ucap * 64u;
  else ops += ((ucap + 3u) & ~3u) * ((PL_LOWCAP + 31u) / 32u) + 16u;
  uint32_t b = 256u + L * 2u * 3u + (L + 16u) * 2u + ucap * 2u * 4u + ucap * 4u * 2u + PL_MAXH * ucap +
               NRQ_MAX_FREE * PL_MAXH + wprcap * npad * 4u * 2u + npad * 2u + 16u + ops * 4u +
               Mcap * 4u + (nlost_cap + 1u) * 8u + nlost_cap * PL_PATCH_STRIDE * 2u + 1024u;
  return pl_r16(b);
}

struct PlanCtx {
  rq_params p;
  const uint8_t *kc;
  const nrq_kconst_hdr *kh;
  const uint32_t *b_rptr, *b_cptr, *b_state;
  const uint16_t *b_cidx, *b_ridx, *b_erow, *b_chead;
  const uint8_t *G, *GT;
  nrq_planjob job;
  const uint32_t *lost, *rep_esi;
  pl_shared *sh;
  uint32_t qcap, lowcap, sh_bytes;
  uint16_t *qmem;
  uint32_t *partial;
  uint8_t *gjmem;
  SB_MEM uint16_t *queue(uint32_t pq) const { uint16_t *q = qmem + (size_t)pq * qcap; PL_ASSUME_LDS(q); return q; }
  SB_MEM uint16_t *claim_l() const { uint16_t *q = qmem + 2u * (size_t)qcap; PL_ASSUME_LDS(q); return q; }
  SB_MEM uint16_t *claim_c() const { uint16_t *q = qmem + 3u * (size_t)qcap; PL_ASSUME_LDS(q); return q; }
  SB_MEM uint32_t *ring() const { uint32_t *q = reinterpret_cast<uint32_t *>(qmem + 2u * (size_t)qcap); PL_ASSUME_LDS(q); return q; }
  SB_MEM uint32_t *part() const { uint32_t *q = partial; PL_ASSUME_LDS(q); return q; }
  SB_MEM uint8_t *gj_flag() const { uint8_t *q = gjmem; PL_ASSUME_LDS(q); return q; }
  SB_MEM uint8_t *gj_used() const { uint8_t *q = gjmem + lowcap; PL_ASSUME_LDS(q); return q; }
  SB_MEM uint32_t *pcbits() const { if (p.L > 16u * lowcap) return nullptr; uint32_t *q = reinterpret_cast<uint32_t *>(gjmem); PL_ASSUME_LDS(q); return q; }
  uint8_t *lds_dyn;
  uint32_t lds_dyn_bytes;
  uint8_t *dense_lds;
  uint32_t dense_bytes;
  uint8_t *aux_lds;
  uint32_t aux_bytes;
  uint32_t Mcap, npcap, ucap;
  pl_work_layout wl;
  uint8_t *work;
  uint32_t *rowstate, *rowinfo, *colinfo;
  uint32_t *pk_cnt, *pk_un, *pk_pa, *pk_vb;
#ifdef PL_STAMP
  unsigned long long st_prev;
  bool st_on;
  bool st_blk;
#endif
  bool collev_hbm;
  uint32_t *cls_glob;
  uint32_t *nrec_ptr;
  uint32_t *wentry;
  uint32_t *own_ptr;
  uint16_t *chk;
  uint16_t *patch_of, *patch_cols, *pc_rows, *pc_head, *ucol;
  uint32_t *emit_bkt;
  bool pcfill_lds;
  uint8_t *patch_len;
  uint32_t *pc_ptr, *pc_fill, *wrows, *lev_ops, *lev_base, *lev_fill, *pivdeg, *lowdeg, *lev_fin, *red_row,
      *red_x, *rec_word, *rec_idx;
  uint16_t *rec_g, *cand;
  uint32_t reccap;
  uint8_t *arena;
  nrq_plan_hdr *hdr;
  uint16_t *pivslot, *pivcol, *colslot, *pivof, *uslot, *lowslot, *pivx, *freex_out;
  uint32_t *fbits;
  uint8_t *mh, *hinv;
  uint32_t off_pivslot, off_pivcol, off_colslot, off_pivof, off_uslot, off_lowslot, off_pivx, off_fbits, off_mh,
      off_freex, off_hinv, fixed_end;
  nrq_job *jobout;
};

#if defined(__HIP_DEVICE_COMPILE__)
#define PL_HBM(T, v) ((T *)(__attribute__((address_space(1))) T *)(uintptr_t)(v))
#else
#define PL_HBM(T, v) (reinterpret_cast<T *>(v))
#endif
SB_HD void pl_ctx_setup(PlanCtx &c, const rq_params &prm, const uint8_t *kc, const nrq_planjob &job, pl_shared *sh,
                        uint8_t *lds_dyn, uint32_t lds_dyn_bytes, uint32_t Mcap, uint32_t npcap, uint32_t ucap,
                        nrq_job *jobout, uint32_t qcap = PL_QCAP, uint32_t lowcap = PL_LOWCAP, uint32_t nt = PL_NT) {
  c.qcap = qcap; c.lowcap = lowcap;
  c.sh_bytes = pl_shared_bytes(qcap, lowcap, nt);
  {
    uint8_t *t = reinterpret_cast<uint8_t *>(sh) + pl_r16((uint32_t)sizeof(pl_shared));
    c.qmem = reinterpret_cast<uint16_t *>(t); t += pl_r16(qcap * 8u);
    c.partial = reinterpret_cast<uint32_t *>(t); t += pl_r16(nt * 4u);
    c.gjmem = t;
  }
  c.kc = kc;
  c.kh = reinterpret_cast<const nrq_kconst_hdr *>(kc);
// ... 2295 lines not shown
  if (i >= c.job.nrep_avail || sh->nextra >= PL_EXTRA_ROWS) { sh->status = PL_FAIL_SINGULAR; return; }
  const uint32_t esi = c.rep_esi[i];
  if (esi < p.K || esi >= (1u << 24)) { sh->status = PL_FAIL_SINGULAR; return; }
  const uint32_t row = sh->M, j = sh->nlow;
  if (row + 1u > c.Mcap || i + 1u > c.npcap || j + 1u > c.lowcap) { (sh->fail_site = __LINE__, sh->status = PL_FAIL_CAPACITY); return; }
  uint32_t cols[RQ_MAX_LT_COLS];
  const uint32_t n = rq_lt_columns(&p, esi + (p.Kp - p.K), cols);
  uint16_t *dst = c.patch_cols + (size_t)i * PL_PATCH_STRIDE;
  uint32_t *ops = reinterpret_cast<uint32_t *>(c.arena + sh->off_ops);
  for (uint32_t k = 0; k < n; k++) {
    dst[k] = (uint16_t)cols[k];
    const uint32_t info = c.colinfo[cols[k]];
    if ((info >> 30) == PL_ST_PIVOT) {
      if (sh->spare_fill >= PL_SPARE_ROWS * NRQ_ROW) { (sh->fail_site = __LINE__, sh->status = PL_FAIL_CAPACITY); return; }
      *pl_op_at(ops, sh->spare_base, sh->spare_fill++) = NRQ_OP(row, c.pivslot[info & 0x3FFFFFFFu]);
    }
  }
  c.patch_len[i] = (uint8_t)n;
  c.patch_of[row] = (uint16_t)i;
  c.rowinfo[row] = PL_UNASSIGNED | PL_PATCHED;
  c.lowslot[j] = (uint16_t)row;
  c.gj_used()[j] = 0;
  sh->M = row + 1u; sh->npatch = i + 1u; sh->nlow = j + 1u; sh->nextra++;
  sh->cand[0] = sh->cand[1] = sh->cand[2] = PL_NONE;
}
template <int Z> SB_HD void pl_extra_b(PlanCtx &c, uint32_t tid, uint32_t nt) {
  pl_shared *sh = c.sh; PL_ASSUME_LDS(sh);
  if (sh->status) return;
  const uint32_t wpr = sh->wpr, rowlen = sh->rowlen, j = sh->nlow - 1u, row = c.lowslot[j];
  if (tid >= rowlen) return;
  uint32_t acc = 0;
  if (tid < wpr) {
    const uint16_t *cols;
    const uint32_t n = pl_row(c, row, &cols);
    for (uint32_t k = 0; k < n; k++) {
      const uint32_t info = c.colinfo[cols[k]], idx = info & 0x3FFFFFFFu;
      if ((info >> 30) == PL_ST_INACT) { if ((idx >> 5) == tid) acc ^= 1u << (idx & 31u); }
      else acc ^= c.wrows[(size_t)c.pivslot[idx] * wpr + tid];
    }
    c.wrows[(size_t)row * wpr + tid] = acc;
  } else {
    acc = ((tid - wpr) == (j >> 5)) ? (1u << (j & 31u)) : 0u;
  }
  sh->xrow[tid] = acc;
}
template <int Z> SB_HD void pl_extra_c(PlanCtx &c, uint32_t tid, uint32_t nt) {
  pl_shared *sh = c.sh; PL_ASSUME_LDS(sh);
  if (sh->status) return;
  const uint32_t rowlen = sh->rowlen, j = sh->nlow - 1u;
  if (tid >= rowlen) return;
  uint32_t *Mb = pl_mb(c);
  uint32_t acc = sh->xrow[tid];
  for (uint32_t q = 0; q < sh->r2; q++) {
    const uint32_t x = c.red_x[q];
    if ((sh->xrow[x >> 5] >> (x & 31u)) & 1u) acc ^= Mb[(size_t)c.red_row[q] * rowlen + tid];
  }
  Mb[(size_t)j * rowlen + tid] = acc;
}
template <int Z> SB_HD void pl_extra_d(PlanCtx &c, uint32_t tid, uint32_t nt) {
  pl_shared *sh = c.sh; PL_ASSUME_LDS(sh);
  if (sh->status || tid != 0) return;
  const uint32_t *row = pl_mb(c) + (size_t)(sh->nlow - 1u) * sh->rowlen;
  sh->xcol = PL_NONE;
  const uint32_t nf = sh->nfree < NRQ_MAX_FREE ? sh->nfree : NRQ_MAX_FREE;
  for (uint32_t f = 0; f < nf; f++) {
    const uint32_t x = sh->freex[f];
    if ((row[x >> 5] >> (x & 31u)) & 1u) {
      sh->xcol = x;
      for (uint32_t g = f; g + 1u < nf; g++) sh->freex[g] = sh->freex[g + 1u];
      sh->nfree--;
      break;
    }
  }
}

template <int Z> SB_HD void pl_mark_failed(PlanCtx &c, uint32_t tid, uint32_t nt) {
  if (tid == 0) (c.sh->fail_site = __LINE__, c.sh->status = PL_FAIL_CAPACITY);
}

SB_HD bool pl_need_wanted(const PlanCtx &c) {
  return (c.job.mode & 0xFFu) == 0u && c.job.inter == 0u && c.sh->npiv != 0u &&
         (c.sh->M + 31u) / 32u * 4u <= 4u * c.qcap;
}
SB_HD uint32_t *pl_need_marks(const PlanCtx &c) { uint32_t *q = reinterpret_cast<uint32_t *>(c.claim_l()); PL_ASSUME_LDS(q); return q; }
template <int Z> SB_HD void pl_final_a(PlanCtx &c, uint32_t tid, uint32_t nt) {
  pl_shared *sh = c.sh; PL_ASSUME_LDS(sh);
  if (sh->status) return;
  const rq_params &p = c.p;
  const uint32_t n_hd = p.Kp + p.S, u = p.L - sh->npiv;
  for (uint32_t col = tid; col < ((n_hd + 7u) & ~7u); col += nt) c.pivof[col] = NRQ_NOSLOT;
  if (tid == 0) {
    sh->tmp0 = (sh->npiv + 63u) & ~63u;
  }
  pl_for_batched(tid, nt, sh->M, [&](uint32_t r) { return c.rowinfo[r]; }, [&](uint32_t r, uint32_t info) {
    if (!(info & PL_UNASSIGNED)) return;
    uint32_t x = PL_ATOM_ADD(&sh->uslot_fill, 1u);
    if (x < u) { c.uslot[x] = (uint16_t)r; c.colslot[c.ucol[x]] = (uint16_t)r; }
  });
}
template <int Z> SB_HD void pl_final_b(PlanCtx &c, uint32_t tid, uint32_t nt) {
  pl_shared *sh = c.sh; PL_ASSUME_LDS(sh);
  if (sh->status) return;
  struct CS { uint32_t col, slot; };
#if defined(__HIP_DEVICE_COMPILE__)
  const uint32_t n_hd8 = (c.p.Kp + c.p.S + 7u) & ~7u, Lp = (c.p.L + 7u) & ~7u;
  if (c.dense_lds && (Lp + n_hd8) * 2u <= c.dense_bytes) {
    uint16_t *cs = reinterpret_cast<uint16_t *>(c.dense_lds), *po = cs + Lp;
    PL_ASSUME_LDS(cs); PL_ASSUME_LDS(po);
    const uint32_t u = c.p.L - sh->npiv;
    for (uint32_t col = tid; col < n_hd8; col += nt) po[col] = NRQ_NOSLOT;
    for (uint32_t col = tid; col < Lp; col += nt) cs[col] = 0;
    __syncthreads();
    for (uint32_t x = tid; x < u; x += nt) cs[c.ucol[x]] = c.uslot[x];
    pl_for_batched(tid, nt, sh->npiv, [&](uint32_t k) { return CS{c.pivcol[k], c.pivslot[k]}; },
                   [&](uint32_t, CS v) { cs[v.col] = (uint16_t)v.slot; if (v.col < n_hd8) po[v.col] = (uint16_t)v.slot; });
    __syncthreads();
    for (uint32_t col = tid; col < c.p.L; col += nt) c.colslot[col] = cs[col];
    for (uint32_t col = tid; col < n_hd8; col += nt) c.pivof[col] = po[col];
  } else
#endif
  pl_for_batched(tid, nt, sh->npiv, [&](uint32_t k) { return CS{c.pivcol[k], c.pivslot[k]}; },
                 [&](uint32_t, CS v) { c.colslot[v.col] = (uint16_t)v.slot; c.pivof[v.col] = (uint16_t)v.slot; });
  if (tid == 0) {
    const rq_params &p = c.p;
    const uint32_t nl = c.job.nlost;
    uint32_t o = sh->arena_top;
    c.part()[0] = o; o = pl_r16(o + sh->wpr * sh->tmp0 * 4u);
    c.part()[1] = o; o = pl_r16(o + sh->M * 4u);
    c.part()[2] = o; o = pl_r16(o + (nl + 1u) * 4u);
    c.part()[3] = o; o = pl_r16(o + nl * 4u + 4u);
    c.part()[4] = o; o = pl_r16(o + nl * PL_PATCH_STRIDE * 2u + NRQ_STORE_SLACK);
    const uint32_t need = pl_need_wanted(c);
    c.part()[5] = need ? o : 0u; if (need) o = pl_r16(o + sh->tmp0 * 2u);
    c.part()[6] = need ? o : 0u; if (need) o = pl_r16(o + sh->wpr * sh->tmp0 * 4u);
    c.part()[7] = need;
    sh->arena_top = o;
    if (o > c.job.arena_cap) (sh->fail_site = __LINE__, sh->status = PL_FAIL_CAPACITY);
    sh->tmp1 = 0;
    (void)p;
  }
}
template <int Z> SB_HD void pl_final_c(PlanCtx &c, uint32_t tid, uint32_t nt) {
  pl_shared *sh = c.sh; PL_ASSUME_LDS(sh);
  if (sh->status) return;
  const rq_params &p = c.p;
  const uint32_t wpr = sh->wpr, stride = sh->tmp0, nl = c.job.nlost;
  uint32_t *wt = reinterpret_cast<uint32_t *>(c.arena + c.part()[0]);
  if (!sh->defer_wt)
    for (uint32_t e = tid; e < wpr * stride; e += nt) {
      const uint32_t w = e / stride, k = e - w * stride;
      wt[e] = k < sh->npiv ? c.wrows[(size_t)c.pivslot[k] * wpr + w] : 0u;
    }
  uint32_t *rowsrc = reinterpret_cast<uint32_t *>(c.arena + c.part()[1]);
  pl_for_batched(tid, nt, sh->M, [&](uint32_t r) { return (uint32_t)c.patch_of[r]; }, [&](uint32_t r, uint32_t pi) {
    uint32_t v = NRQ_ROW_ZERO;
    if (pi != 0xFFFFu) v = NRQ_ROW_REP | pi;
    else if (r >= p.S + p.H && r < p.S + p.H + p.K) v = r - p.S - p.H;
    rowsrc[r] = v;
  });
  uint32_t *cptr = reinterpret_cast<uint32_t *>(c.arena + c.part()[2]);
  uint32_t *orow = reinterpret_cast<uint32_t *>(c.arena + c.part()[3]);
  uint16_t *osl = reinterpret_cast<uint16_t *>(c.arena + c.part()[4]);
  uint8_t *lenq = pl_lenq(c);
  const bool in_lds = nl <= 2u * c.qcap;
  struct ED { uint32_t e, dg; };
  pl_for_batched(tid, nt, nl, [&](uint32_t g) { const uint32_t e = c.lost[g]; return ED{e, c.b_rptr[p.S + p.H + e + 1] - c.b_rptr[p.S + p.H + e]}; },
                 [&](uint32_t g, ED v) {
                   if (in_lds) lenq[g] = (uint8_t)v.dg;
                   else { c.pivdeg[g] = v.dg; orow[g] = v.e; }
                 });
  if (in_lds && tid < 3u && nl + tid < ((nl + 3u) & ~3u)) lenq[nl + tid] = 0;
  (void)cptr; (void)osl;
  uint32_t ops = 0;
  pl_for_batched(tid, nt, sh->nlev + 2u, [&](uint32_t l) { return c.lev_ops[l]; }, [&](uint32_t, uint32_t v) { ops += v; });
  if (ops) PL_ATOM_ADD(&sh->tmp1, ops);
}
template <int Z> SB_HD void pl_final_c2(PlanCtx &c, uint32_t tid, uint32_t nt) {
  pl_shared *sh = c.sh; PL_ASSUME_LDS(sh);
  const uint32_t nl = c.job.nlost;
  if (sh->status || nl <= 2u * c.qcap) return;
  const uint32_t per = (nl + nt - 1u) / nt, a = tid * per < nl ? tid * per : nl, b = a + per < nl ? a + per : nl;
  uint32_t sum = 0;
  for (uint32_t g0 = a; g0 < b; g0 += PL_BATCH) {
    uint32_t v[PL_BATCH];
#pragma unroll
    for (uint32_t j = 0; j < PL_BATCH; j++) v[j] = c.pivdeg[g0 + j < b ? g0 + j : g0];
#pragma unroll
    for (uint32_t j = 0; j < PL_BATCH; j++) if (g0 + j < b) sum += v[j];
  }
  reinterpret_cast<uint32_t *>(c.queue(0u))[tid] = sum;
}
template <int Z> SB_HD void pl_final_c3(PlanCtx &c, uint32_t tid, uint32_t nt) {
  pl_shared *sh = c.sh; PL_ASSUME_LDS(sh);
  if (sh->status || c.job.nlost <= 2u * c.qcap || tid != 0) return;
  uint32_t *ps = reinterpret_cast<uint32_t *>(c.queue(0u));
  uint32_t run = 0;
  for (uint32_t t = 0; t < nt; t++) { const uint32_t v = ps[t]; ps[t] = run; run += v; }
  ps[nt] = run;
}
template <int Z> SB_HD void pl_final_d(PlanCtx &c, uint32_t tid, uint32_t nt) {
  pl_shared *sh = c.sh; PL_ASSUME_LDS(sh);
  const rq_params &p = c.p;
  if (!sh->status && c.job.nlost <= 2u * c.qcap) {
    const uint32_t nl = c.job.nlost;
    uint32_t *cptr = reinterpret_cast<uint32_t *>(c.arena + c.part()[2]);
    uint32_t *orow = reinterpret_cast<uint32_t *>(c.arena + c.part()[3]);
    for (uint32_t g = tid; g < nl; g += nt) {
      uint32_t pos, off;
      pl_len_rank(c, g, nl, pos, off);
      cptr[pos] = off; orow[pos] = c.lost[g]; c.pivdeg[g] = off;
    }
    if (tid == 0) cptr[nl] = pl_len_total(c, nl);
  } else if (!sh->status) {
    const uint32_t nl = c.job.nlost, per = (nl + nt - 1u) / nt, a = tid * per < nl ? tid * per : nl, b = a + per < nl ? a + per : nl;
    const uint32_t *ps = reinterpret_cast<const uint32_t *>(c.queue(0u));
    uint32_t *cptr = reinterpret_cast<uint32_t *>(c.arena + c.part()[2]);
    uint32_t run = ps[tid];
    for (uint32_t g0 = a; g0 < b; g0 += PL_BATCH) {
      uint32_t v[PL_BATCH];
#pragma unroll
      for (uint32_t j = 0; j < PL_BATCH; j++) v[j] = c.pivdeg[g0 + j < b ? g0 + j : g0];
#pragma unroll
      for (uint32_t j = 0; j < PL_BATCH; j++) if (g0 + j < b) { cptr[g0 + j] = run; run += v[j]; }
    }
    if (tid == 0) cptr[nl] = ps[nt];
  }
  if (!sh->status && c.part()[7])
    for (uint32_t i = tid; i < (sh->M + 31u) / 32u; i += nt) pl_need_marks(c)[i] = 0u;
  if (tid != 0) return;
  nrq_plan_hdr h;
  memset(&h, 0, sizeof(h));
  h.magic = NRQ_PLAN_MAGIC;
  h.status = sh->status ? 1u : 0u;
  h.reserved[0] = sh->status;
  h.reserved[1] = sh->nextra;
  h.fail_site = sh->fail_site;
  h.K = p.Kp; h.Kp = p.Kp; h.S = p.S; h.H = p.H; h.W = p.W; h.L = p.L; h.P = p.P; h.B = p.B;
  h.M = sh->M; h.npiv = sh->npiv; h.u = p.L - sh->npiv; h.nlow = sh->nlow; h.r2 = sh->r2; h.nfree = sh->nfree;
  h.nlev = sh->nlev; h.nrows = sh->nrows; h.pipe = NRQ_PIPE; h.wpr = sh->wpr;
  h.npiv_pad = sh->tmp0;
  h.off_ops = sh->off_ops; h.off_pivslot = c.off_pivslot; h.off_pivcol = c.off_pivcol; h.off_wt = c.part()[0];
  h.off_lowslot = c.off_lowslot; h.off_pivx = c.off_pivx; h.off_fbits = c.off_fbits; h.off_mh = c.off_mh;
  h.off_freex = c.off_freex; h.off_hinv = c.off_hinv; h.off_colslot = c.off_colslot; h.off_pivof = c.off_pivof;
  h.off_uslot = c.off_uslot; h.total_bytes = sh->arena_top;
  h.off_augt = sh->off_augt; h.lpr = pl_bin_in_stream(p.L) ? 0u : sh->lpr; h.aug_stride = sh->aug_stride;
  if (!sh->status) {
    const uint32_t nl = c.job.nlost;
    uint32_t *cptr = reinterpret_cast<uint32_t *>(c.arena + c.part()[2]);
    uint32_t run = 0;
    if (nl <= 2u * c.qcap) run = pl_len_total(c, nl);
    else run = reinterpret_cast<const uint32_t *>(c.queue(0u))[nt];
    (void)cptr;
    h.n_xor_ops = sh->tmp1 + run + sh->spare_fill;
  }
  *c.hdr = h;
  if (c.job.hdr_out) *PL_HBM(nrq_plan_hdr, c.job.hdr_out) = h;
  if (c.jobout) {
    nrq_job j;
    memset(&j, 0, sizeof(j));
    j.plan = (uint64_t)(uintptr_t)c.arena;
    if (!sh->status) {
      j.rowsrc = (uint64_t)(uintptr_t)(c.arena + c.part()[1]);
      j.src = c.job.src; j.rep = c.job.rep; j.inter = c.job.inter; j.out = c.job.src;
      j.out_cptr = (uint64_t)(uintptr_t)(c.arena + c.part()[2]);
      j.out_row = (uint64_t)(uintptr_t)(c.arena + c.part()[3]);
      j.out_slots = (uint64_t)(uintptr_t)(c.arena + c.part()[4]);
      j.nout = c.job.nlost;
    }
    *c.jobout = j;
  }
}

SB_HD void pl_wt_fill(uint8_t *arena, const uint32_t *wrows, uint32_t e0, uint32_t step) {
  const nrq_plan_hdr *h = reinterpret_cast<const nrq_plan_hdr *>(arena);
  if (h->status) return;
  const uint32_t wpr = h->wpr, stride = h->npiv_pad, npiv = h->npiv;
  const uint16_t *pivslot = reinterpret_cast<const uint16_t *>(arena + h->off_pivslot);
  uint32_t *wt = reinterpret_cast<uint32_t *>(arena + h->off_wt);
  for (uint32_t e = e0; e < wpr * stride; e += step) {
    const uint32_t w = e / stride, k = e - w * stride;
    wt[e] = k < npiv ? wrows[(size_t)pivslot[k] * wpr + w] : 0u;
  }
  if (!h->off_needslot) return;
  const uint32_t pad = h->need_pad, nneed = h->nneed;
  const uint16_t *nslot = reinterpret_cast<const uint16_t *>(arena + h->off_needslot);
  uint32_t *wneed = reinterpret_cast<uint32_t *>(arena + h->off_wneed);
  for (uint32_t e = e0; e < wpr * pad; e += step) {
    const uint32_t w = e / pad, j = e - w * pad;
    wneed[e] = j < nneed ? wrows[(size_t)nslot[j] * wpr + w] : 0u;
  }
}

template <int Z> SB_HD void pl_final_e(PlanCtx &c, uint32_t tid, uint32_t nt) {
  pl_shared *sh = c.sh; PL_ASSUME_LDS(sh);
  if (sh->status) return;
  const rq_params &p = c.p;
  const uint32_t nl = c.job.nlost;
  const uint32_t *cptr = reinterpret_cast<const uint32_t *>(c.arena + c.part()[2]);
  uint16_t *osl = reinterpret_cast<uint16_t *>(c.arena + c.part()[4]);
  uint32_t *marks = c.part()[7] ? pl_need_marks(c) : nullptr;
  for (uint32_t g = tid; g < nl; g += nt) {
    const uint32_t e = c.lost[g], a = c.b_rptr[p.S + p.H + e], n = c.b_rptr[p.S + p.H + e + 1] - a;
    const uint32_t o = nl <= 2u * c.qcap ? c.pivdeg[g] : cptr[g];
    constexpr uint32_t CB = 8;
    for (uint32_t k0 = 0; k0 < n; k0 += CB) {
      uint32_t col[CB], sl[CB];
#pragma unroll
      for (uint32_t q = 0; q < CB; q++) col[q] = k0 + q < n ? c.b_cidx[a + k0 + q] : 0u;
#pragma unroll
      for (uint32_t q = 0; q < CB; q++) sl[q] = c.colslot[col[q]];
#pragma unroll
      for (uint32_t q = 0; q < CB; q++)
        if (k0 + q < n) {
          osl[o + k0 + q] = (uint16_t)sl[q];
          if (marks) PL_ATOM_OR(&marks[sl[q] >> 5], 1u << (sl[q] & 31u));
        }
    }
  }
}

#define PL_NEED_UNIT 64u
SB_HD bool pl_need_marked(const PlanCtx &c, uint32_t k, uint32_t end) {
  if (k >= end) return false;
  const uint32_t s = c.pivslot[k];
  return ((pl_need_marks(c)[s >> 5] >> (s & 31u)) & 1u) != 0u;
}
template <int Z> SB_HD void pl_need_a(PlanCtx &c, uint32_t tid, uint32_t nt) {
  pl_shared *sh = c.sh; PL_ASSUME_LDS(sh);
  if (sh->status || !c.part()[7]) return;
  const uint32_t unit = tid / PL_NEED_UNIT, nunit = nt / PL_NEED_UNIT, np = sh->npiv;
  const uint32_t per = ((np + nunit - 1u) / nunit + PL_NEED_UNIT - 1u) / PL_NEED_UNIT * PL_NEED_UNIT;
  const uint32_t a = unit * per < np ? unit * per : np, b = a + per < np ? a + per : np;
  uint32_t n = 0;
#if defined(__HIP_DEVICE_COMPILE__)
  for (uint32_t k0 = a; k0 < b; k0 += PL_NEED_UNIT) n += (uint32_t)__popcll(__ballot(pl_need_marked(c, k0 + (tid & 63u), b)));
#else
  if (tid % PL_NEED_UNIT) return;
  for (uint32_t k = a; k < b; k++) n += pl_need_marked(c, k, b) ? 1u : 0u;
#endif
  if (tid % PL_NEED_UNIT == 0u) c.part()[8u + unit] = n;
}
template <int Z> SB_HD void pl_need_b(PlanCtx &c, uint32_t tid, uint32_t nt) {
  pl_shared *sh = c.sh; PL_ASSUME_LDS(sh);
  if (sh->status || !c.part()[7]) return;
  const uint32_t unit = tid / PL_NEED_UNIT, nunit = nt / PL_NEED_UNIT, np = sh->npiv, wpr = sh->wpr;
  const uint32_t per = ((np + nunit - 1u) / nunit + PL_NEED_UNIT - 1u) / PL_NEED_UNIT * PL_NEED_UNIT;
  const uint32_t a = unit * per < np ? unit * per : np, b = a + per < np ? a + per : np;
  const uint32_t *cnt = c.part() + 8u;
  uint32_t base = 0, nneed = 0;
  for (uint32_t v = 0; v < nunit; v++) { const uint32_t x = cnt[v]; base += v < unit ? x : 0u; nneed += x; }
  const uint32_t pad = (nneed + 63u) & ~63u;
  uint16_t *nslot = reinterpret_cast<uint16_t *>(c.arena + c.part()[5]);
  uint32_t *wneed = reinterpret_cast<uint32_t *>(c.arena + c.part()[6]);
#if defined(__HIP_DEVICE_COMPILE__)
  for (uint32_t k0 = a; k0 < b; k0 += PL_NEED_UNIT) {
    const uint32_t k = k0 + (tid & 63u);
    const bool on = pl_need_marked(c, k, b);
    const unsigned long long m = __ballot(on);
    const uint32_t j = base + (uint32_t)__popcll(m & ((1ull << (tid & 63u)) - 1ull));
    base += (uint32_t)__popcll(m);
#else
  for (uint32_t k = a; k < b && tid % PL_NEED_UNIT == 0u; k++) {
    const bool on = pl_need_marked(c, k, b);
    const uint32_t j = base;
    base += on ? 1u : 0u;
#endif
    if (!on) continue;
    const uint32_t s = c.pivslot[k];
    nslot[j] = (uint16_t)s;
    if (!sh->defer_wt)
      for (uint32_t w = 0; w < wpr; w++) wneed[(size_t)w * pad + j] = c.wrows[(size_t)s * wpr + w];
  }
  if (!sh->defer_wt)
    for (uint32_t e = tid; e < (pad - nneed) * wpr; e += nt) wneed[(size_t)(e / (pad - nneed)) * pad + nneed + e % (pad - nneed)] = 0u;
  if (tid == 0) {
    nrq_plan_hdr *h = c.hdr;
    h->nneed = nneed; h->need_pad = pad; h->off_needslot = c.part()[5]; h->off_wneed = c.part()[6];
    if (c.job.hdr_out) {
      nrq_plan_hdr *ho = PL_HBM(nrq_plan_hdr, c.job.hdr_out);
      ho->nneed = nneed; ho->need_pad = pad; ho->off_needslot = c.part()[5]; ho->off_wneed = c.part()[6];
    }
  }
}

#endif
```

nanorq_amd/csrc/planner_seq.h:

```cpp
{
  pl_shared *sh_ = c.sh;
  if (PL_SEG != 2 && PL_SEG != 4) {
  PL_PHASE(pl_init_a);
  PL_PHASE(pl_init_b);
  PL_PHASE(pl_scan_a);
  PL_PHASE(pl_scan_b);
  PL_PHASE(pl_scan_c);
  PL_PHASE(pl_pcsc_fill);
  {
    const uint32_t guard_max = 4u * c.p.L + 64u;
    uint32_t rd_ = 0;
    for (;;) {
      PL_ST(c, 0);
      const uint32_t st_ = sh_->status, nv_ = sh_->nV, nq_ = sh_->nq[rd_ & 1u];
      if (st_ + nv_ + nq_ != 0x12345u) PL_ST(c, 1);
      PL_STEER_SYNC;
      PL_ST(c, 2);
      if (st_ != 0 || nv_ == 0 || rd_ >= guard_max) break;
#ifdef PL_TRACE_ROUND
      PL_TRACE_ROUND(nq_, nv_);
#endif
      if (PL_LIKELY(nq_ > 0)) {
        PL_PHASE1_CLAIM(pl_round_claim, rd_);
        PL_ST(c, 8);
// ... 93 lines not shown
      PL_STEER_SYNC;
      if (rev_) PL_PHASE(pl_mhrev_scatter);
      else
      for (uint32_t tl_ = 0; tl_ * PL_MH_TILE < sh_->npiv; tl_++) {
        PL_PHASE1(pl_mh_load, tl_);
        PL_PHASE1(pl_mh_acc, tl_);
      }
    } else {
      PL_PHASE(pl_mh_fetch);
    }
    PL_PHASE(pl_low_c);
    {
      const uint32_t u_ = c.p.L - sh_->npiv;
      const bool wave_ = PL_GJ_WAVE && pl_gjw_ok(c);
      if (wave_ || pl_gj_blocked(c, PL_NT_)) {
        for (uint32_t w_ = 0; w_ * 32u < u_; w_++) {
          if (wave_) PL_PHASE1(pl_gjp_wave, w_);
          else {
          PL_PHASE1(pl_gjp_init, w_);
          for (uint32_t x_ = w_ * 32u; x_ < u_ && x_ < w_ * 32u + 32u; x_++) {
            PL_PHASE1(pl_gjp_bid, x_);
            PL_PHASE1(pl_gjp_step, x_);
          }
          PL_PHASE1(pl_gjp_comb, w_);
          }
          PL_PHASE1(pl_gjp_stage, w_);
          PL_PHASE1(pl_gjp_apply, w_);
        }
      } else {
      if (u_) PL_PHASE1(pl_gj_a, 0u);
      for (uint32_t x_ = 0; x_ < u_; x_++) {
        const uint32_t a_ = x_ | (x_ + 1u < u_ ? 0x80000000u : 0u);
        PL_PHASE1(pl_gj_b, a_);
      }
      }
    }
    for (uint32_t try_ = 0; try_ <= PL_EXTRA_ROWS + 1u; try_++) {
      PL_PHASE(pl_dense_a);
      PL_PHASE(pl_dense_b);
      const bool solve_ = sh_->status == 0 && sh_->dense_ok;
      const uint32_t nf_ = sh_->nfree;
      PL_STEER_SYNC;
      if (solve_) {
        for (uint32_t f_ = 0; f_ < nf_; f_++) {
          PL_PHASE1(pl_dense_step_a, f_);
          PL_PHASE1(pl_dense_step_b, f_);
        }
      }
      const bool done_ = sh_->status != 0 || sh_->dense_ok;
      PL_STEER_SYNC;
      if (done_) break;
      PL_PHASE(pl_extra_a);
      const bool stop_ = sh_->status != 0;
      PL_STEER_SYNC;
      if (stop_) break;
      PL_PHASE(pl_extra_b);
      PL_PHASE(pl_extra_c);
      PL_PHASE(pl_extra_d);
      const uint32_t xc_ = sh_->xcol;
      PL_STEER_SYNC;
      if (xc_ != PL_NONE) {
        PL_PHASE1(pl_gj_a, xc_);
        PL_PHASE1(pl_gj_b, xc_);
      }
    }
    PL_PHASE(pl_dense_c);
    PL_PHASE(pl_bin_a);
    PL_PHASE(pl_bin_b);
    PL_PHASE(pl_bin_c);
    PL_PHASE(pl_final_a);
    PL_PHASE(pl_final_b);
    PL_PHASE(pl_final_c);
    PL_PHASE(pl_final_c2);
    PL_PHASE(pl_final_c3);
    }
  } else if (st2_ == 0 && PL_SEG != 1 && PL_SEG != 3 && PL_SEG != 4) {
    PL_PHASE(pl_mark_failed);
  }
  if (PL_SEG != 1 && PL_SEG != 3 && PL_SEG != 4) {
    PL_PHASE(pl_final_d);
    PL_PHASE(pl_final_e);
    PL_PHASE(pl_need_a);
    PL_PHASE(pl_need_b);
  }
}
```

nanorq_amd/csrc/solve_body.h:

```cpp
#ifndef NRQ_SOLVE_BODY_H
#define NRQ_SOLVE_BODY_H

#include <stdint.h>
#include <string.h>

#include "plan.h"

#if defined(__HIPCC__)
#define SB_HD __host__ __device__ __forceinline__
#define SB_MEM __host__ __device__ __forceinline__
#else
#define SB_HD static inline
#define SB_MEM inline
struct uint2 { uint32_t x, y; };
struct uint4 { uint32_t x, y, z, w; };
#endif

#if defined(__HIP_DEVICE_COMPILE__)
#define NRQ_GAS __attribute__((address_space(1)))
#else
#define NRQ_GAS
#endif
template <class X> SB_HD const NRQ_GAS X *gptr(const void *p) { return (const NRQ_GAS X *)p; }
template <class X> SB_HD const NRQ_GAS X *gptr(uint64_t p) { return (const NRQ_GAS X *)(uintptr_t)p; }
template <class X> SB_HD NRQ_GAS X *gptr_w(uint64_t p) { return (NRQ_GAS X *)(uintptr_t)p; }

typedef struct nrq_job {
  uint64_t plan;
  uint64_t rowsrc;
  uint64_t src;
  uint64_t rep;
  uint64_t inter;
  uint64_t out;
  uint64_t out_cptr;
  uint64_t out_slots;
  uint64_t out_row;
  uint32_t nout;
  uint32_t pad;
} nrq_job;

#if defined(__HIP_DEVICE_COMPILE__)
#undef NRQ_WAVE_ANY
#define NRQ_WAVE_ANY(x) (__ballot(x) != 0ull)
#elif !defined(NRQ_WAVE_ANY)
#define NRQ_WAVE_ANY(x) (x)
#endif
#if defined(__HIP_DEVICE_COMPILE__)
#ifdef NRQ_NO_UNIFORM
__device__ __forceinline__ uint32_t nrq_uniform(uint32_t x) { return x; }
#else
__device__ __forceinline__ uint32_t nrq_uniform(uint32_t x) { return (uint32_t)__builtin_amdgcn_readfirstlane((int)x); }
#endif
template <class P> __device__ __forceinline__ P nrq_uniform_ptr(P p) {
  const uint64_t v = (uint64_t)(uintptr_t)p;
  const uint64_t u = (uint64_t)nrq_uniform((uint32_t)v) | ((uint64_t)nrq_uniform((uint32_t)(v >> 32)) << 32);
  return (P)(uintptr_t)u;
}
#else
SB_HD uint32_t nrq_uniform(uint32_t x) { return x; }
template <class P> SB_HD P nrq_uniform_ptr(P p) { return p; }
#endif
#if defined(__HIP_DEVICE_COMPILE__)
#define NRQ_SCHED_FENCE() __builtin_amdgcn_sched_barrier(0)
#else
#define NRQ_SCHED_FENCE() do { } while (0)
#endif
#if defined(__HIP_DEVICE_COMPILE__)
#define NRQ_MARK(c, i) do { if ((c).dbg && (c).dbg_t0) (c).dbg[i] = (unsigned long long)clock64(); } while (0)
#define NRQ_MARK_MAX(c, i) do { if ((c).dbg) atomicMax(&(c).dbg[i], (unsigned long long)clock64()); } while (0)
#else
#define NRQ_MARK(c, i) do { } while (0)
#define NRQ_MARK_MAX(c, i) do { } while (0)
#endif
#define NRQ_ROW_ZERO 0xFFFFFFFFu
#define NRQ_ROW_REP 0x80000000u

template <int WB> struct SV {
  static constexpr int ND = (WB + 3) / 4;
  uint32_t w[ND];
};

template <int WB> struct SVAlign { static constexpr uintptr_t mask = (uintptr_t)(WB == 12 ? 3 : WB - 1); };
struct nrq_u3 { uint32_t x, y, z; };
#ifndef NRQ_W12_GROUP
#define NRQ_W12_GROUP 8u
#endif
SB_HD constexpr uint32_t nrq_group_strips(uint32_t wbe) { return wbe >= 128u ? 1u : wbe == 12u ? NRQ_W12_GROUP : 128u / wbe; }
template <int WB> SB_HD SV<WB> sv_zero() {
  SV<WB> r;
#pragma unroll
  for (int i = 0; i < SV<WB>::ND; i++) r.w[i] = 0;
  return r;
}
template <int WB> SB_HD void sv_xor(SV<WB> &a, const SV<WB> &b) {
#pragma unroll
  for (int i = 0; i < SV<WB>::ND; i++) a.w[i] ^= b.w[i];
}
template <int WB> SB_HD void sv_xor_masked(SV<WB> &a, const SV<WB> &b, uint32_t mask) {
#pragma unroll
  for (int i = 0; i < SV<WB>::ND; i++) a.w[i] ^= b.w[i] & mask;
}
SB_HD uint32_t xtime32(uint32_t x) {
  const uint32_t hi = x & 0x80808080u;
  return ((x ^ hi) << 1) ^ ((hi - (hi >> 7)) & 0x1d1d1d1du);
}
SB_HD uint32_t nrq_xor3(uint32_t a, uint32_t b, uint32_t c) {
#if defined(__HIP_DEVICE_COMPILE__)
  return __builtin_amdgcn_bitop3_b32(a, b, c, 0x96);
#else
  return a ^ b ^ c;
#endif
}
SB_HD uint32_t nrq_xor_and(uint32_t a, uint32_t b, uint32_t c) {
#if defined(__HIP_DEVICE_COMPILE__)
  return __builtin_amdgcn_bitop3_b32(a, b, c, 0x78);
#else
  return a ^ (b & c);
#endif
}
template <int WB> SB_HD SV<WB> sv_xtime(const SV<WB> &a) {
  SV<WB> r;
#pragma unroll
// ... 1080 lines not shown
  const NRQ_GAS uint8_t *hinv = c.template arr<uint8_t>(c.h->off_hinv);
  const uint32_t H = c.h->H, nfree = c.h->nfree;
  const uint32_t hq = tid & 15u;
  if (hq >= H) return;
  if constexpr (BATCH) {
    const uint32_t nparts = nt >> 4;
    for (uint32_t f0 = tid >> 4; f0 < nfree; f0 += 8u * nparts) {
      uint32_t coef[8];
#pragma unroll
      for (uint32_t i = 0; i < 8; i++) coef[i] = hinv[(size_t)(f0 + i * nparts < nfree ? f0 + i * nparts : f0) * H + hq];
      const SV<WB> r = lds_get<WB, G>(c.slots(), c.h->S + hq);
#pragma unroll
      for (uint32_t i = 0; i < 8; i++) {
        const uint32_t f = f0 + i * nparts;
        if (f >= nfree || !coef[i]) continue;
        SV<WB> t = sv_mul<WB>(r, coef[i]);
        lds_xor<WB, G>(c.cf(), f, t);
      }
    }
    return;
  }
  for (uint32_t f = tid >> 4; f < nfree; f += nt >> 4) {
    uint32_t coef = hinv[(size_t)f * H + hq];
    if (!coef) continue;
    SV<WB> t = sv_mul<WB>(lds_get<WB, G>(c.slots(), c.h->S + hq), coef);
    lds_xor<WB, G>(c.cf(), f, t);
  }
}

template <int WB, int G = 1, bool BATCH = false> SB_HD void ph_dense_cu(const StripCtx<WB, G> &c, uint32_t tid, uint32_t nt) {
  const NRQ_GAS uint16_t *pivx = c.template arr<uint16_t>(c.h->off_pivx);
  const NRQ_GAS uint32_t *fbits = c.template arr<uint32_t>(c.h->off_fbits);
  const NRQ_GAS uint16_t *freex = c.template arr<uint16_t>(c.h->off_freex);
  uint32_t fx0 = 0, px0 = 0;
  if constexpr (BATCH) {
    if (tid < c.h->nfree) fx0 = freex[tid];
    if (tid < c.h->r2) px0 = pivx[tid];
  }
  for (uint32_t p = tid; p < c.h->r2; p += nt) {
    SV<WB> v = lds_get<WB, G>(c.slots(), c.h->M + p);
    uint32_t fb = fbits[p];
    while (fb) {
      uint32_t f = (uint32_t)__builtin_ctz(fb);
      fb &= fb - 1u;
      SV<WB> t = lds_get<WB, G>(c.cf(), f);
      sv_xor<WB>(v, t);
    }
    lds_put<WB, G>(c.cu(), (BATCH && p == tid) ? px0 : (uint32_t)pivx[p], v);
  }
  for (uint32_t f = tid; f < c.h->nfree; f += nt) lds_put<WB, G>(c.cu(), (BATCH && f == tid) ? fx0 : (uint32_t)freex[f], lds_get<WB, G>(c.cf(), f));
}

template <int WB, int G = 1> SB_HD SV<WB> t4_get(const uint8_t *t4, uint32_t e) {
  if constexpr (WB == 12) {
    SV<12> r = sv_zero<12>();
    const uint4 v = reinterpret_cast<const uint4 *>(t4)[e];
    r.w[0] = v.x; r.w[1] = v.y; r.w[2] = v.z;
    return r;
  } else return lds_get<WB, G>(t4, e);
}
template <int WB, int G = 1> SB_HD void t4_put(uint8_t *t4, uint32_t e, const SV<WB> &v) {
  if constexpr (WB == 12) {
    uint4 t; t.x = v.w[0]; t.y = v.w[1]; t.z = v.w[2]; t.w = 0u;
    reinterpret_cast<uint4 *>(t4)[e] = t;
  } else lds_put<WB, G>(t4, e, v);
}
template <int WB, int G = 1> SB_HD void ph_tables(const StripCtx<WB, G> &c, uint32_t tid, uint32_t nt) {
  const uint32_t ngroups = c.h->wpr * 8u, u = c.h->u;
  for (uint32_t e = tid; e < ngroups * 16u; e += nt) {
    uint32_t grp = e >> 4, nib = e & 15u;
    SV<WB> v = sv_zero<WB>();
#pragma unroll
    for (uint32_t bq = 0; bq < 4; bq++) {
      uint32_t x = grp * 4u + bq;
      if (((nib >> bq) & 1u) && x < u) {
        SV<WB> t = lds_get<WB, G>(c.cu(), x);
        sv_xor<WB>(v, t);
      }
    }
    t4_put<WB, G>(c.t4(), e, v);
  }
}

template <int WB, int NW, int G = 1, bool FAST = true>
SB_HD void backsub_one(const StripCtx<WB, G> &c, const uint8_t *t4, uint32_t slot, const uint32_t (&bitsw)[NW],
                       uint32_t wpr) {
  SV<WB> acc = lds_get<WB, G>(c.slots(), slot);
#pragma unroll
  for (uint32_t w = 0; w < (uint32_t)NW; w++) {
    if (w >= wpr) break;
    const uint32_t bits = bitsw[w];
#if defined(__HIP_DEVICE_COMPILE__)
    if constexpr (WB == 16 && G == 1) {
      uint32_t odd = bits & 0xF0F0F0F0u, even = (bits << 4) & 0xF0F0F0F0u;
      asm volatile("" : "+v"(odd), "+v"(even));
      if constexpr (FAST) {
      const uint32_t tbw = (uint32_t)(uintptr_t)t4 + w * 2048u;
      uint4 d[8];
#pragma unroll
      for (uint32_t q = 0; q < 8; q++) d[q] = *NRQ_LDSP(uint4, t4_addr(tbw, (q & 1u) ? odd : even, q >> 1) + q * 256u);
#pragma unroll
      for (uint32_t q = 0; q < 8; q += 2) {
        acc.w[0] = nrq_xor3(acc.w[0], d[q].x, d[q + 1].x); acc.w[1] = nrq_xor3(acc.w[1], d[q].y, d[q + 1].y);
        acc.w[2] = nrq_xor3(acc.w[2], d[q].z, d[q + 1].z); acc.w[3] = nrq_xor3(acc.w[3], d[q].w, d[q + 1].w);
      }
      } else {
        const uint32_t tb = (uint32_t)(uintptr_t)t4;
#pragma unroll
      for (uint32_t q = 0; q < 8; q++) {
        const uint32_t a = t4_addr(tb, (q & 1u) ? odd : even, q >> 1) + (w * 8u + q) * 256u;
        const uint4 v = *NRQ_LDSP(uint4, a);
        acc.w[0] ^= v.x; acc.w[1] ^= v.y; acc.w[2] ^= v.z; acc.w[3] ^= v.w;
        if (q == 3) NRQ_SCHED_FENCE();
      }
      }
      NRQ_SCHED_FENCE();
      continue;
    }
    if constexpr (WB == 8 && G == 1) {
      uint32_t odd = (bits >> 1) & 0x78787878u, even = (bits << 3) & 0x78787878u;
      asm volatile("" : "+v"(odd), "+v"(even));
      const uint32_t tbw = (uint32_t)(uintptr_t)t4 + w * 1024u;
      uint2 d[8];
#pragma unroll
      for (uint32_t q = 0; q < 8; q++) d[q] = *NRQ_LDSP(uint2, t4_addr(tbw, (q & 1u) ? odd : even, q >> 1) + q * 128u);
#pragma unroll
      for (uint32_t q = 0; q < 8; q += 2) {
        acc.w[0] = nrq_xor3(acc.w[0], d[q].x, d[q + 1].x); acc.w[1] = nrq_xor3(acc.w[1], d[q].y, d[q + 1].y);
      }
      NRQ_SCHED_FENCE();
      continue;
    }
    if constexpr (WB == 12 && G == 1) {
      uint32_t odd = bits & 0xF0F0F0F0u, even = (bits << 4) & 0xF0F0F0F0u;
      asm volatile("" : "+v"(odd), "+v"(even));
      const uint32_t tbw = (uint32_t)(uintptr_t)t4 + w * 2048u;
      uint4 d[8];
#pragma unroll
      for (uint32_t q = 0; q < 8; q++) d[q] = *NRQ_LDSP(uint4, t4_addr(tbw, (q & 1u) ? odd : even, q >> 1) + q * 256u);
      uint32_t pad = 0;
#pragma unroll
      for (uint32_t q = 0; q < 8; q += 2) {
        acc.w[0] = nrq_xor3(acc.w[0], d[q].x, d[q + 1].x); acc.w[1] = nrq_xor3(acc.w[1], d[q].y, d[q + 1].y);
        acc.w[2] = nrq_xor3(acc.w[2], d[q].z, d[q + 1].z); pad = nrq_xor3(pad, d[q].w, d[q + 1].w);
      }
      asm volatile("" : : "v"(pad));
      NRQ_SCHED_FENCE();
      continue;
    }
#endif
#pragma unroll
    for (uint32_t q = 0; q < 8; q++) {
      const uint32_t nib = (bits >> (4u * q)) & 15u;
      SV<WB> t = t4_get<WB, G>(t4, (w * 8u + q) * 16u + nib);
      sv_xor<WB>(acc, t);
      if (q == 3) NRQ_SCHED_FENCE();
    }
    NRQ_SCHED_FENCE();
  }
  lds_put<WB, G>(c.slots(), slot, acc);
}

#define NRQ_BACKSUB_VIEW(c, need)                                                                                            \
  const NRQ_GAS uint16_t *pivslot = (c).template arr<uint16_t>((need) ? (c).h->off_needslot : (c).h->off_pivslot);      \
  const NRQ_GAS uint32_t *wt = (c).template arr<uint32_t>((need) ? (c).h->off_wneed : (c).h->off_wt);                   \
  const uint32_t stride = (need) ? (c).h->need_pad : (c).h->npiv_pad, npiv = (need) ? (c).h->nneed : (c).h->npiv
template <int WB, int NW, int G = 1, bool FAST = true>
SB_HD void backsub_fixed(const StripCtx<WB, G> &c, bool need, uint32_t tid, uint32_t nt) {
  if constexpr (!FAST) {

  NRQ_BACKSUB_VIEW(c, need);
  const uint32_t wpr = c.h->wpr;
  const uint8_t *t4 = c.t4();
  for (uint32_t k = tid; k < npiv; k += 2 * nt) {
    const uint32_t k2 = k + nt;
    uint32_t a[NW], b[NW];
    const uint32_t sa = pivslot[k];
    const uint32_t sb = k2 < npiv ? pivslot[k2] : 0u;
#pragma unroll
    for (uint32_t w = 0; w < (uint32_t)NW; w++) a[w] = w < wpr ? wt[(size_t)w * stride + k] : 0u;
#pragma unroll
    for (uint32_t w = 0; w < (uint32_t)NW; w++) b[w] = (w < wpr && k2 < npiv) ? wt[(size_t)w * stride + k2] : 0u;
    backsub_one<WB, NW, G, false>(c, t4, sa, a, wpr);
    if (k2 < npiv) backsub_one<WB, NW, G, false>(c, t4, sb, b, wpr);
  }
    return;
  }
  NRQ_BACKSUB_VIEW(c, need);
  const uint32_t wpr = c.h->wpr;
  const uint8_t *t4 = c.t4();
  uint32_t a[NW], b[NW], sa = 0, sb = 0;
  uint32_t k = tid;
  if (k < npiv) {
    sa = pivslot[k];
#pragma unroll
    for (uint32_t w = 0; w < (uint32_t)NW; w++) a[w] = w < wpr ? wt[(size_t)w * stride + k] : 0u;
  }
  for (; k < npiv; k += 2 * nt) {
    const uint32_t k2 = k + nt, k3 = k + 2 * nt;
    if (k2 < npiv) {
      sb = pivslot[k2];
#pragma unroll
      for (uint32_t w = 0; w < (uint32_t)NW; w++) b[w] = w < wpr ? wt[(size_t)w * stride + k2] : 0u;
    }
    backsub_one<WB, NW, G, FAST>(c, t4, sa, a, wpr);
    if (k3 < npiv) {
      sa = pivslot[k3];
#pragma unroll
      for (uint32_t w = 0; w < (uint32_t)NW; w++) a[w] = w < wpr ? wt[(size_t)w * stride + k3] : 0u;
    }
    if (k2 < npiv) backsub_one<WB, NW, G, FAST>(c, t4, sb, b, wpr);
  }
}

template <int WB, int G = 1, bool FAST = true> SB_HD void ph_backsub(const StripCtx<WB, G> &c, uint32_t tid, uint32_t nt) {
  const uint32_t wpr = c.h->wpr;
  const bool need = c.job->inter == 0 && c.h->off_needslot != 0u;
  if (wpr <= 4) backsub_fixed<WB, 4, G, FAST>(c, need, tid, nt);
  else if (wpr <= 8) backsub_fixed<WB, 8, G, FAST>(c, need, tid, nt);
  else if (wpr <= 12) backsub_fixed<WB, 12, G, FAST>(c, need, tid, nt);
  else if (wpr <= 24) backsub_fixed<WB, 24, G, FAST>(c, need, tid, nt);
  else {
    NRQ_BACKSUB_VIEW(c, need);
    const uint8_t *t4 = c.t4();
    for (uint32_t k = tid; k < npiv; k += nt) {
      uint32_t s = pivslot[k];
      SV<WB> acc = lds_get<WB, G>(c.slots(), s);
      for (uint32_t w = 0; w < wpr; w++) {
        uint32_t bits = wt[(size_t)w * stride + k];
#pragma unroll
        for (uint32_t q = 0; q < 8; q++) {
          uint32_t nib = (bits >> (4u * q)) & 15u;
          SV<WB> t = t4_get<WB, G>(t4, (w * 8u + q) * 16u + nib);
          sv_xor<WB>(acc, t);
        }
      }
      lds_put<WB, G>(c.slots(), s, acc);
    }
  }
}

template <int WB, int G = 1> SB_HD void ph_park(const StripCtx<WB, G> &c, uint32_t tid, uint32_t nt) {
  const NRQ_GAS uint16_t *uslot = c.template arr<uint16_t>(c.h->off_uslot);
  for (uint32_t x = tid; x < c.h->u; x += nt) lds_put<WB, G>(c.slots(), uslot[x], lds_get<WB, G>(c.cu(), x));
}

#ifndef NRQ_STORE_CHUNK
#define NRQ_STORE_CHUNK 8u
#endif
#ifndef NRQ_STORE_TRIP
#define NRQ_STORE_TRIP 32u
#endif
#define NRQ_STORE_SLACK (16u + NRQ_STORE_TRIP * 4u)
#define NRQ_LT_LIST_MAX 33u
static_assert(NRQ_LT_LIST_MAX <= 2u * NRQ_STORE_TRIP, "ph_store reads at most two trips of a list; out_slots[] slack is sized for that");
#define NRQ_STORE_TRIPS_MAX ((NRQ_LT_LIST_MAX + NRQ_STORE_TRIP - 1u) / NRQ_STORE_TRIP)
static_assert(NRQ_STORE_SLACK >= 2u * (NRQ_STORE_TRIPS_MAX * NRQ_STORE_TRIP - 1u),
              "the bytes behind out_slots[] do not cover ph_store's reads past a last list of one entry in a wave with a list of NRQ_LT_LIST_MAX");
template <int WB, int G = 1> SB_HD uint32_t out_elems(const nrq_job *job, const nrq_plan_hdr *h) { return (job->inter ? h->L : 0u) + job->nout; }
SB_HD void store_trip(const NRQ_GAS uint16_t *osl, uint32_t e, uint32_t end, uint32_t (&raw)[NRQ_STORE_TRIP / 2u]) {
  (void)end;
#ifdef __HIP_DEVICE_COMPILE__
  typedef uint32_t u4 __attribute__((ext_vector_type(4)));
  typedef u4 u4a __attribute__((aligned(2)));
#pragma unroll
  for (uint32_t k = 0; k < NRQ_STORE_TRIP / 8u; k++) {
    const u4 w = *reinterpret_cast<const NRQ_GAS u4a *>(osl + e + 8u * k);
    raw[4u * k] = w.x; raw[4u * k + 1u] = w.y; raw[4u * k + 2u] = w.z; raw[4u * k + 3u] = w.w;
  }
#elif defined(NRQ_STORE_TRIP_UNBOUNDED)
#pragma unroll
  for (uint32_t k = 0; k < NRQ_STORE_TRIP / 8u; k++) memcpy(&raw[4u * k], osl + e + 8u * k, 16);
#else
#pragma unroll
  for (uint32_t k = 0; k < NRQ_STORE_TRIP / 2u; k++)
    raw[k] = (e + 2u * k < end ? (uint32_t)osl[e + 2u * k] : 0u) | (e + 2u * k + 1u < end ? (uint32_t)osl[e + 2u * k + 1u] : 0u) << 16;
#endif
}
SB_HD uint32_t store_slot(const uint32_t (&raw)[NRQ_STORE_TRIP / 2u], uint32_t k, uint32_t e, uint32_t end, uint32_t zero_at) {
  return e + k < end ? ((raw[k / 2u] >> (16u * (k & 1u))) & 0xFFFFu) + NRQ_SCRATCH : zero_at;
}
template <int WB, int G = 1, bool FAST = true> SB_HD void ph_store(const StripCtx<WB, G> &c, NRQ_GAS uint8_t *ostage, uint32_t tid, uint32_t nt) {
  constexpr int STB = 8;
  const NRQ_GAS uint16_t *colslot = c.template arr<uint16_t>(c.h->off_colslot);
  const uint32_t L = c.h->L, ni = c.job->inter ? L : 0u;
  for (uint32_t base = tid; base < ni; base += STB * nt) {
    uint32_t sl[STB];
#pragma unroll
    for (int q = 0; q < STB; q++) {
      uint32_t col = base + (uint32_t)q * nt;
      sl[q] = col < L ? colslot[col] : 0u;
    }
#pragma unroll
    for (int q = 0; q < STB; q++) {
      uint32_t col = base + (uint32_t)q * nt;
      if (col < L) g_put_stream<WB>(ostage + (size_t)col * (WB * G), WB, lds_get<WB, G>(c.slots(), sl[q]));
    }
  }
  const NRQ_GAS uint32_t *cptr = gptr<uint32_t>(c.job->out_cptr);
  const NRQ_GAS uint16_t *osl = gptr<uint16_t>(c.job->out_slots);
  if constexpr (FAST) {
  const uint32_t nout = c.job->nout;
  constexpr uint32_t CH = NRQ_STORE_CHUNK;
  const uint32_t zero_at = tid & (NRQ_SCRATCH - 1u);
  uint32_t e_n = 0, end_n = 0;
  if (tid < nout) { e_n = cptr[tid]; end_n = cptr[tid + 1]; }
  const uint32_t npass = (nout + nt - 1u) / nt;
  for (uint32_t pass = 0, q = tid; pass < npass; pass++, q += nt) {
    uint32_t e = e_n;
    const uint32_t end = end_n;
    e_n = end_n = 0;
    if (q + nt < nout) { e_n = cptr[q + nt]; end_n = cptr[q + nt + 1]; }
    SV<WB> acc = sv_zero<WB>();
    while (NRQ_WAVE_ANY(e < end)) {
      constexpr uint32_t TR = NRQ_STORE_TRIP;
      uint32_t raw[TR / 2u];
      store_trip(osl, e, end, raw);
#pragma unroll
      for (uint32_t k0 = 0; k0 < TR; k0 += CH) {
        if (k0 && !NRQ_WAVE_ANY(e + k0 < end)) break;
        SV<WB> v[CH];
#pragma unroll
        for (uint32_t k = 0; k < CH; k++) v[k] = lds_get<WB, G>(c.lds, store_slot(raw, k0 + k, e, end, zero_at));
#pragma unroll
        for (uint32_t k = 0; k + 1u < CH; k += 2u)
#pragma unroll
          for (int i = 0; i < SV<WB>::ND; i++) acc.w[i] = nrq_xor3(acc.w[i], v[k].w[i], v[k + 1u].w[i]);
      }
      e += TR;
    }
    if (q < nout) g_put_stream<WB>(ostage + (size_t)(ni + q) * (WB * G), WB, acc);
  }
  } else {
  const uint32_t nout = c.job->nout;
  constexpr uint32_t CH = 32u;
  uint32_t e_n = 0, end_n = 0;
  if (tid < nout) { e_n = cptr[tid]; end_n = cptr[tid + 1]; }
  for (uint32_t q = tid; q < nout; q += nt) {
    uint32_t e = e_n;
    const uint32_t end = end_n;
    if (q + nt < nout) { e_n = cptr[q + nt]; end_n = cptr[q + nt + 1]; }
    SV<WB> acc = sv_zero<WB>();
    while (e < end) {
      uint32_t sl[CH];
#pragma unroll
      for (uint32_t k = 0; k < CH; k++) sl[k] = e + k < end ? (uint32_t)osl[e + k] : NRQ_NOSLOT;
#pragma unroll
      for (uint32_t k = 0; k < CH; k++)
        if (sl[k] != NRQ_NOSLOT) sv_xor<WB>(acc, lds_get<WB, G>(c.slots(), sl[k]));
      e += CH;
    }
    g_put_stream<WB>(ostage + (size_t)(ni + q) * (WB * G), WB, acc);
  }
  }
}
template <int WB, int G = 1> SB_HD void ph_store_raw(const StripCtx<WB, G> &c, NRQ_GAS uint8_t *ostage, uint32_t tid, uint32_t nt) {
  const uint32_t M = c.h->M, u = c.h->u;
  constexpr int STB = 4;
  for (uint32_t base = tid; base < M + u; base += STB * nt) {
    SV<WB> v[STB];
#pragma unroll
    for (int q = 0; q < STB; q++) {
      const uint32_t i = base + (uint32_t)q * nt;
      v[q] = i < M ? lds_get<WB, G>(c.slots(), i) : i < M + u ? lds_get<WB, G>(c.cu(), i - M) : sv_zero<WB>();
    }
#pragma unroll
    for (int q = 0; q < STB; q++) {
      const uint32_t i = base + (uint32_t)q * nt;
      if (i < M + u) g_put_stream<WB>(ostage + (size_t)i * (WB * G), WB, v[q]);
    }
  }
}
template <int WB> struct GroupDst {
  NRQ_GAS uint8_t *inter, *out;
  const NRQ_GAS uint32_t *orow;
  uint32_t ni, nout, T, strip0, nstrips;
  uint32_t lsub;
};
template <int WB, int G, bool PIPELINED, int AL> SB_HD void pf_scatter_impl(const GroupDst<WB> &g, const NRQ_GAS uint8_t *ostage, size_t stage_stride, uint32_t u0,
                                        uint32_t u1, uint32_t p, uint32_t np, uint32_t sub) {
  const uint32_t lsub = g.lsub, pmask = (1u << lsub) - 1u;
  if constexpr (WB == 12 && AL == 1) {
    if ((g.strip0 + (1u << lsub)) * 12u > g.T) { pf_scatter_impl<WB, G, PIPELINED, 2>(g, ostage, stage_stride, u0, u1, p, np, sub); return; }
  }
#ifndef NRQ_SCATTER_PB
#define NRQ_SCATTER_PB 4
#endif
#ifndef NRQ_SCATTER_PUT
#define NRQ_SCATTER_PUT g_put
#endif
#ifndef NRQ_W12_SCATTER_PB
#define NRQ_W12_SCATTER_PB NRQ_SCATTER_PB
#endif
  constexpr int PB = WB == 12 ? NRQ_W12_SCATTER_PB : NRQ_SCATTER_PB;
  if constexpr (!PIPELINED) {
  for (uint32_t base = u0 + p; base < u1; base += PB * np) {
      SV<WB> v[PB];
      uint32_t row[PB];
  #pragma unroll
      for (int q = 0; q < PB; q++) {
        const uint32_t u = base + (uint32_t)q * np, i = u >> lsub;
        row[q] = (u < u1 && i >= g.ni) ? g.orow[i - g.ni] : i;
        v[q] = u < u1 ? g_get_l2<WB>(ostage + (size_t)(u & pmask) * stage_stride + (size_t)i * (WB * G) + sub * WB) : sv_zero<WB>();
      }
  #pragma unroll
      for (int q = 0; q < PB; q++) {
        const uint32_t u = base + (uint32_t)q * np, i = u >> lsub, strip = g.strip0 + (u & pmask);
        if (u >= u1 || strip >= g.nstrips) continue;
        if constexpr (AL != 0) {
          if constexpr (AL == 2) { const uint32_t rem = g.T - strip * WB; g_put_al12((i < g.ni ? g.inter : g.out) + (size_t)row[q] * g.T + (size_t)strip * WB, rem < 12u ? rem : 12u, v[q]); }
          else g_put_al<WB>((i < g.ni ? g.inter : g.out) + (size_t)row[q] * g.T + (size_t)strip * WB, v[q]);
        } else if constexpr (G == 1) {
          const uint32_t rem = g.T - strip * WB;
          NRQ_GAS uint8_t *dst = (i < g.ni ? g.inter : g.out) + (size_t)row[q] * g.T + (size_t)strip * WB;
          NRQ_SCATTER_PUT<WB>(dst, rem < (uint32_t)WB ? rem : (uint32_t)WB, v[q]);
        } else {
          const uint32_t at = strip * (WB * G) + sub * WB;
          if (at >= g.T) continue;
          const uint32_t rem = g.T - at;
          NRQ_GAS uint8_t *dst = (i < g.ni ? g.inter : g.out) + (size_t)row[q] * g.T + at;
          NRQ_SCATTER_PUT<WB>(dst, rem < (uint32_t)WB ? rem : (uint32_t)WB, v[q]);
        }
      }
    }
    return;
  }
  const uint32_t first = u0 + p, step = (uint32_t)PB * np;
  if (first >= u1) return;
  SV<WB> v[PB], vn[PB];
  uint32_t row[PB], rown[PB];
  auto load = [&](uint32_t base, SV<WB> (&vv)[PB], uint32_t (&rr)[PB]) {
#pragma unroll
    for (int q = 0; q < PB; q++) {
      const uint32_t u = base + (uint32_t)q * np, i = u >> lsub;
      rr[q] = (u < u1 && i >= g.ni) ? g.orow[i - g.ni] : i;
      vv[q] = u < u1 ? g_get_l2<WB>(ostage + (size_t)(u & pmask) * stage_stride + (size_t)i * (WB * G) + sub * WB) : sv_zero<WB>();
    }
// ... 64 lines not shown
```

Measured before the change: 1643.

## Skip back-substitution by folding pivot weight rows into per-output view

```diff
diff --git a/__graft_entry__.py b/__graft_entry__.py
--- a/__graft_entry__.py
+++ b/__graft_entry__.py
@@ -27,6 +27,7 @@
     nbuild.build_shape_emu()
     nbuild.build_launch_emu()
     nbuild.build_out_lists_emu()
+    nbuild.build_out_view_emu()
     nbuild.build_model_lib()
     nbuild.build_rows_probe()
     nbuild.build_tools()
diff --git a/include/nanorq_hip.h b/include/nanorq_hip.h
--- a/include/nanorq_hip.h
+++ b/include/nanorq_hip.h
@@ -32,6 +32,7 @@
   uint32_t plan_segmented;
   uint32_t backsub_strip;
   uint32_t encplan_device;
+  uint32_t out_view;
 } nrq_call_stats;
 
 int nrq_ctx_create(int device, void *stream, nrq_ctx **out);
diff --git a/nanorq_amd/binding.py b/nanorq_amd/binding.py
--- a/nanorq_amd/binding.py
+++ b/nanorq_amd/binding.py
@@ -28,7 +28,7 @@
                 ("wg_waves_per_simd", C.c_uint32), ("host_planned", C.c_uint32), ("movers_aligned", C.c_uint32),
                 ("plan_ahead", C.c_uint32), ("strip_bytes_b", C.c_uint32), ("blocks_b", C.c_uint32),
                 ("plan_wg_threads", C.c_uint32), ("plan_compact_state", C.c_uint32), ("plan_segmented", C.c_uint32),
-                ("backsub_strip", C.c_uint32), ("encplan_device", C.c_uint32)]
+                ("backsub_strip", C.c_uint32), ("encplan_device", C.c_uint32), ("out_view", C.c_uint32)]
 
     def as_dict(self):
         return {k: getattr(self, k) for k, _ in self._fields_}
@@ -198,7 +198,8 @@
 PLAN_FIELDS = ("magic status K Kp J S H W L P P1 B M npiv u nlow r2 nfree nlev nrows pipe wpr "
                "npiv_pad n_xor_ops off_ops off_pivslot off_pivcol off_wt off_lowslot off_pivx off_fbits "
                "off_mh off_freex off_hinv off_colslot off_pivof off_uslot total_bytes reserved0 reserved1 fail_site "
-               "off_augt lpr aug_stride nneed need_pad off_needslot off_wneed").split()
+               "off_augt lpr aug_stride nneed need_pad off_needslot off_wneed off_wout out_pad out_n off_out_cptr "
+               "off_out_slots").split()
 
 
 def params(K):
diff --git a/nanorq_amd/build.py b/nanorq_amd/build.py
--- a/nanorq_amd/build.py
+++ b/nanorq_amd/build.py
@@ -25,6 +25,7 @@
 JEMU = os.path.join(ROOT, "tests", "emu", "librxset_runs_emu.so")
 NEMU = os.path.join(ROOT, "tests", "emu", "liblaunch_emu.so")
 UEMU = os.path.join(ROOT, "tests", "emu", "libout_lists_emu.so")
+VEMU = os.path.join(ROOT, "tests", "emu", "libout_view_emu.so")
 MODEL = os.path.join(ROOT, "tests", "emu", "libnanorq_model.so")
 ROWS = os.path.join(ROOT, "tests", "gpu", "librows_probe.so")
 
@@ -132,6 +133,10 @@
 
 def build_out_lists_emu(force=False):
     return _build_emu(UEMU, os.path.join(ROOT, "tests", "emu", "out_lists_emu.cpp"), ("out_lists.h", "rq_math.h"), force)
+
+
+def build_out_view_emu(force=False):
+    return _build_emu(VEMU, os.path.join(ROOT, "tests", "emu", "out_view_emu.cpp"), ("out_lists.h", "plan.h", "rq_math.h"), force)
 
 
 def build_ingest_emu(force=False):
@@ -280,6 +285,7 @@
     build_shape_emu(force="-f" in sys.argv)
     build_launch_emu(force="-f" in sys.argv)
     build_out_lists_emu(force="-f" in sys.argv)
+    build_out_view_emu(force="-f" in sys.argv)
     build_model_lib(force="-f" in sys.argv)
     build_rows_probe(force="-f" in sys.argv)
     build_tools(force="-f" in sys.argv)
diff --git a/nanorq_amd/csrc/nrq_device.hip b/nanorq_amd/csrc/nrq_device.hip
--- a/nanorq_amd/csrc/nrq_device.hip
+++ b/nanorq_amd/csrc/nrq_device.hip
@@ -457,6 +457,7 @@
   pl_tag_pl_final_e = 15,
   pl_tag_pl_need_a = 15,
   pl_tag_pl_need_b = 15,
+  pl_tag_pl_out_w = 15,
   pl_tag_pl_mark_failed = 15,
 };
 
@@ -1527,9 +1528,10 @@
     uint32_t plan_bytes = 0;
     std::vector<uint32_t> rowsrc, cptr, orow;
     std::vector<uint16_t> cols;
+    std::vector<uint32_t> wout;
     int state = 0;
     uint32_t used = 0;
-    size_t off_plan = 0, off_rowsrc = 0, off_cptr = 0, off_row = 0, off_cols = 0;
+    size_t off_plan = 0, off_wout = 0, off_rowsrc = 0, off_cptr = 0, off_row = 0, off_cols = 0;
   };
   std::vector<Prep> prep(nblk);
   const uint32_t pad = p.Kp - K;
@@ -1573,6 +1575,7 @@
     }
     build_out_lists(p, reinterpret_cast<const uint16_t *>(pr.plan.p + reinterpret_cast<const nrq_plan_hdr *>(pr.plan.p)->off_colslot),
                     nl, lost, pr.cptr, pr.cols, pr.orow);
+    if (!c.inter) build_out_w(pr.plan.p, pr.cptr, pr.cols, pr.wout);
     for (uint32_t &g : pr.orow) g = lost[g];
     pr.state = 1;
   };
@@ -1610,6 +1613,7 @@
     if (pr.state != 1) continue;
     nsolve++;
     pr.off_plan = off;   off = r16(off + pr.plan_bytes);
+    pr.off_wout = off;   off = r16(off + pr.wout.size() * 4);
     pr.off_rowsrc = off; off = r16(off + pr.rowsrc.size() * 4);
     pr.off_cptr = off;   off = r16(off + pr.cptr.size() * 4);
     pr.off_row = off;    off = r16(off + pr.orow.size() * 4);
@@ -1643,7 +1647,15 @@
       memcpy(hs + pr.off_cptr, pr.cptr.data(), pr.cptr.size() * 4);
       memcpy(hs + pr.off_row, pr.orow.data(), pr.orow.size() * 4);
       if (!pr.cols.empty()) memcpy(hs + pr.off_cols, pr.cols.data(), pr.cols.size() * 2);
-      const nrq_plan_hdr *h = reinterpret_cast<const nrq_plan_hdr *>(hs + pr.off_plan);
+      nrq_plan_hdr *h = reinterpret_cast<nrq_plan_hdr *>(hs + pr.off_plan);
+      if (!pr.wout.empty()) {
+        memcpy(hs + pr.off_wout, pr.wout.data(), pr.wout.size() * 4);
+        h->off_wout = j.out_w = (uint32_t)(pr.off_wout - pr.off_plan);
+        h->out_n = (uint32_t)pr.orow.size(); h->out_pad = (h->out_n + 63u) & ~63u;
+        h->total_bytes = h->off_wout + (uint32_t)pr.wout.size() * 4u;
+        ctx->stats.out_view++;
+        ctx->stats.plan_bytes += pr.wout.size() * 4;
+      }
       hdrs.push_back(h);
       if (ctx->stats.npiv == 0) {
         ctx->stats.npiv = h->npiv; ctx->stats.u = h->u; ctx->stats.nlev = h->nlev; ctx->stats.nfree = h->nfree;
@@ -1895,6 +1907,7 @@
       }
       ctx->stats.xor_ops += hd[b].n_xor_ops;
       ctx->stats.plan_bytes += hd[b].total_bytes;
+      if (hd[b].off_wout) ctx->stats.out_view++;
     } else if (hd[b].reserved[0] == PL_FAIL_CAPACITY) {
       if (ctx->tune.prof || ctx->tune.diag) fprintf(stderr, "[NRQ_PROF] block %u: device planner capacity exceeded at planner_body.h:%u (npiv %u u %u nlev %u nrows %u M %u nlost %u)\n", b, hd[b].fail_site, hd[b].npiv, hd[b].u, hd[b].nlev, hd[b].nrows, hd[b].M, c.h_nlost[b]);
       (*fallback)[b] = 1;
diff --git a/nanorq_amd/csrc/out_lists.h b/nanorq_amd/csrc/out_lists.h
--- a/nanorq_amd/csrc/out_lists.h
+++ b/nanorq_amd/csrc/out_lists.h
@@ -3,6 +3,7 @@
 #include <stdint.h>
 #include <string.h>
 #include <vector>
+#include "plan.h"
 #include "rq_math.h"
 
 inline void build_out_lists(const rq_params &p, const uint16_t *colslot, uint32_t n, const uint32_t *isis,
@@ -33,4 +34,22 @@
   cptr[n] = o;
 }
 
+inline void build_out_w(const uint8_t *plan, const std::vector<uint32_t> &cptr, const std::vector<uint16_t> &cols,
+                        std::vector<uint32_t> &wout) {
+  const nrq_plan_hdr *h = reinterpret_cast<const nrq_plan_hdr *>(plan);
+  const uint32_t n = cptr.empty() ? 0u : (uint32_t)cptr.size() - 1u, wpr = h->wpr, opad = (n + 63u) & ~63u;
+  wout.assign((size_t)wpr * opad, 0u);
+  if (!wpr || !n) return;
+  const uint16_t *pivslot = reinterpret_cast<const uint16_t *>(plan + h->off_pivslot);
+  const uint32_t *wt = reinterpret_cast<const uint32_t *>(plan + h->off_wt);
+  std::vector<uint32_t> pivot_of(h->M + h->r2 + 1u, 0xFFFFFFFFu);
+  for (uint32_t k = 0; k < h->npiv; k++) pivot_of[pivslot[k]] = k;
+  for (uint32_t q = 0; q < n; q++)
+    for (uint32_t e = cptr[q]; e < cptr[q + 1]; e++) {
+      const uint32_t k = pivot_of[cols[e]];
+      if (k == 0xFFFFFFFFu) continue;
+      for (uint32_t w = 0; w < wpr; w++) wout[(size_t)w * opad + q] ^= wt[(size_t)w * h->npiv_pad + k];
+    }
+}
+
 #endif
diff --git a/nanorq_amd/csrc/plan.h b/nanorq_amd/csrc/plan.h
--- a/nanorq_amd/csrc/plan.h
+++ b/nanorq_amd/csrc/plan.h
@@ -103,6 +103,11 @@
   uint32_t need_pad;
   uint32_t off_needslot;
   uint32_t off_wneed;
+  uint32_t off_wout;
+  uint32_t out_pad;
+  uint32_t out_n;
+  uint32_t off_out_cptr;
+  uint32_t off_out_slots;
 } nrq_plan_hdr;
 #ifdef __cplusplus
 static_assert(sizeof(nrq_plan_hdr) <= 256u, "nrq_plan_hdr is read as a 256-byte prefix");
diff --git a/nanorq_amd/csrc/planner_body.h b/nanorq_amd/csrc/planner_body.h
--- a/nanorq_amd/csrc/planner_body.h
+++ b/nanorq_amd/csrc/planner_body.h
@@ -248,7 +248,8 @@
   else ops += ((ucap + 3u) & ~3u) * ((PL_LOWCAP + 31u) / 32u) + 16u;
   uint32_t b = 256u + L * 2u * 3u + (L + 16u) * 2u + ucap * 2u * 4u + ucap * 4u * 2u + PL_MAXH * ucap +
                NRQ_MAX_FREE * PL_MAXH + wprcap * npad * 4u * 2u + npad * 2u + 16u + ops * 4u +
-               Mcap * 4u + (nlost_cap + 1u) * 8u + nlost_cap * PL_PATCH_STRIDE * 2u + 1024u;
+               Mcap * 4u + (nlost_cap + 1u) * 8u + nlost_cap * PL_PATCH_STRIDE * 2u + 1024u +
+               wprcap * ((nlost_cap + 63u) & ~63u) * 4u + 16u;
   return pl_r16(b);
 }
 
@@ -2710,6 +2711,10 @@
   return (c.job.mode & 0xFFu) == 0u && c.job.inter == 0u && c.sh->npiv != 0u &&
          (c.sh->M + 31u) / 32u * 4u <= 4u * c.qcap;
 }
+#define PL_OUTW 24u
+SB_HD bool pl_out_wanted(const PlanCtx &c) {
+  return (c.job.mode & 0xFFu) == 0u && c.job.inter == 0u && c.sh->npiv != 0u && c.sh->wpr != 0u && c.job.nlost != 0u;
+}
 SB_HD uint32_t *pl_need_marks(const PlanCtx &c) { uint32_t *q = reinterpret_cast<uint32_t *>(c.claim_l()); PL_ASSUME_LDS(q); return q; }
 template <int Z> SB_HD void pl_final_a(PlanCtx &c, uint32_t tid, uint32_t nt) {
   pl_shared *sh = c.sh; PL_ASSUME_LDS(sh);
@@ -2762,6 +2767,10 @@
     c.part()[5] = need ? o : 0u; if (need) o = pl_r16(o + sh->tmp0 * 2u);
     c.part()[6] = need ? o : 0u; if (need) o = pl_r16(o + sh->wpr * sh->tmp0 * 4u);
     c.part()[7] = need;
+    const uint32_t opad = (nl + 63u) & ~63u, oend = pl_r16(o + sh->wpr * opad * 4u);
+    const bool outw = pl_out_wanted(c) && o <= c.job.arena_cap && oend <= c.job.arena_cap;
+    c.part()[PL_OUTW] = outw ? o : 0u; c.part()[PL_OUTW + 1u] = outw ? opad : 0u;
+    if (outw) o = oend;
     sh->arena_top = o;
     if (o > c.job.arena_cap) (sh->fail_site = __LINE__, sh->status = PL_FAIL_CAPACITY);
     sh->tmp1 = 0;
@@ -2779,6 +2788,8 @@
       const uint32_t w = e / stride, k = e - w * stride;
       wt[e] = k < sh->npiv ? c.wrows[(size_t)c.pivslot[k] * wpr + w] : 0u;
     }
+  if (c.part()[PL_OUTW])
+    for (uint32_t e = tid; e < (p.L - sh->npiv) * wpr; e += nt) c.wrows[(size_t)c.uslot[e / wpr] * wpr + e % wpr] = 0u;
   uint32_t *rowsrc = reinterpret_cast<uint32_t *>(c.arena + c.part()[1]);
   pl_for_batched(tid, nt, sh->M, [&](uint32_t r) { return (uint32_t)c.patch_of[r]; }, [&](uint32_t r, uint32_t pi) {
     uint32_t v = NRQ_ROW_ZERO;
@@ -2872,6 +2883,10 @@
   h.off_freex = c.off_freex; h.off_hinv = c.off_hinv; h.off_colslot = c.off_colslot; h.off_pivof = c.off_pivof;
   h.off_uslot = c.off_uslot; h.total_bytes = sh->arena_top;
   h.off_augt = sh->off_augt; h.lpr = pl_bin_in_stream(p.L) ? 0u : sh->lpr; h.aug_stride = sh->aug_stride;
+  if (!sh->status && c.part()[PL_OUTW]) {
+    h.off_wout = c.part()[PL_OUTW]; h.out_pad = c.part()[PL_OUTW + 1u]; h.out_n = c.job.nlost;
+    h.off_out_cptr = c.part()[2]; h.off_out_slots = c.part()[4];
+  }
   if (!sh->status) {
     const uint32_t nl = c.job.nlost;
     uint32_t *cptr = reinterpret_cast<uint32_t *>(c.arena + c.part()[2]);
@@ -2894,8 +2909,38 @@
       j.out_row = (uint64_t)(uintptr_t)(c.arena + c.part()[3]);
       j.out_slots = (uint64_t)(uintptr_t)(c.arena + c.part()[4]);
       j.nout = c.job.nlost;
+      j.out_w = c.part()[PL_OUTW];
     }
     *c.jobout = j;
+  }
+}
+
+SB_HD void pl_wout_fill(uint32_t *wout, const uint32_t *cptr, const uint16_t *osl, const uint32_t *wrows, uint32_t wpr, uint32_t nout,
+                        uint32_t opad, uint32_t q0, uint32_t step) {
+  constexpr uint32_t WB = 8, EB = 4;
+  for (uint32_t q = q0; q < opad; q += step) {
+    const uint32_t a = q < nout ? cptr[q] : 0u, b = q < nout ? cptr[q + 1u] : 0u;
+    for (uint32_t w0 = 0; w0 < wpr; w0 += WB) {
+      uint32_t acc[WB];
+#pragma unroll
+      for (uint32_t j = 0; j < WB; j++) acc[j] = 0u;
+      for (uint32_t e = a; e < b; e += EB) {
+        uint32_t s[EB], v[EB][WB];
+#pragma unroll
+        for (uint32_t i = 0; i < EB; i++) s[i] = osl[e + i < b ? e + i : e];
+#pragma unroll
+        for (uint32_t i = 0; i < EB; i++)
+#pragma unroll
+          for (uint32_t j = 0; j < WB; j++) v[i][j] = (e + i < b && w0 + j < wpr) ? wrows[(size_t)s[i] * wpr + w0 + j] : 0u;
+#pragma unroll
+        for (uint32_t i = 0; i < EB; i++)
+#pragma unroll
+          for (uint32_t j = 0; j < WB; j++) acc[j] ^= v[i][j];
+      }
+#pragma unroll
+      for (uint32_t j = 0; j < WB; j++)
+        if (w0 + j < wpr) wout[(size_t)(w0 + j) * opad + q] = acc[j];
+    }
   }
 }
 
@@ -2909,6 +2954,9 @@
     const uint32_t w = e / stride, k = e - w * stride;
     wt[e] = k < npiv ? wrows[(size_t)pivslot[k] * wpr + w] : 0u;
   }
+  if (h->off_wout)
+    pl_wout_fill(reinterpret_cast<uint32_t *>(arena + h->off_wout), reinterpret_cast<const uint32_t *>(arena + h->off_out_cptr),
+                 reinterpret_cast<const uint16_t *>(arena + h->off_out_slots), wrows, wpr, h->out_n, h->out_pad, e0, step);
   if (!h->off_needslot) return;
   const uint32_t pad = h->need_pad, nneed = h->nneed;
   const uint16_t *nslot = reinterpret_cast<const uint16_t *>(arena + h->off_needslot);
@@ -3011,4 +3059,11 @@
   }
 }
 
-#endif
+template <int Z> SB_HD void pl_out_w(PlanCtx &c, uint32_t tid, uint32_t nt) {
+  pl_shared *sh = c.sh; PL_ASSUME_LDS(sh);
+  if (sh->status || !c.part()[PL_OUTW] || sh->defer_wt) return;
+  pl_wout_fill(reinterpret_cast<uint32_t *>(c.arena + c.part()[PL_OUTW]), reinterpret_cast<const uint32_t *>(c.arena + c.part()[2]),
+               reinterpret_cast<const uint16_t *>(c.arena + c.part()[4]), c.wrows, sh->wpr, c.job.nlost, c.part()[PL_OUTW + 1u], tid, nt);
+}
+
+#endif
diff --git a/nanorq_amd/csrc/planner_seq.h b/nanorq_amd/csrc/planner_seq.h
--- a/nanorq_amd/csrc/planner_seq.h
+++ b/nanorq_amd/csrc/planner_seq.h
@@ -199,5 +199,6 @@
     PL_PHASE(pl_final_e);
     PL_PHASE(pl_need_a);
     PL_PHASE(pl_need_b);
+    PL_PHASE(pl_out_w);
   }
 }
diff --git a/nanorq_amd/csrc/solve_body.h b/nanorq_amd/csrc/solve_body.h
--- a/nanorq_amd/csrc/solve_body.h
+++ b/nanorq_amd/csrc/solve_body.h
@@ -36,8 +36,9 @@
   uint64_t out_slots;
   uint64_t out_row;
   uint32_t nout;
-  uint32_t pad;
+  uint32_t out_w;
 } nrq_job;
+SB_HD bool nrq_job_out_view(const nrq_job *job) { return job->out_w != 0u && job->inter == 0; }
 
 #if defined(__HIP_DEVICE_COMPILE__)
 #undef NRQ_WAVE_ANY
@@ -1284,82 +1285,89 @@
   }
 }
 
+template <int WB, int G = 1, bool FAST = true>
+SB_HD void t4_word(SV<WB> &acc, const uint8_t *t4, uint32_t w, uint32_t bits) {
+#if defined(__HIP_DEVICE_COMPILE__)
+  if constexpr (WB == 16 && G == 1) {
+    uint32_t odd = bits & 0xF0F0F0F0u, even = (bits << 4) & 0xF0F0F0F0u;
+    asm volatile("" : "+v"(odd), "+v"(even));
+    if constexpr (FAST) {
+    const uint32_t tbw = (uint32_t)(uintptr_t)t4 + w * 2048u;
+    uint4 d[8];
+#pragma unroll
+    for (uint32_t q = 0; q < 8; q++) d[q] = *NRQ_LDSP(uint4, t4_addr(tbw, (q & 1u) ? odd : even, q >> 1) + q * 256u);
+#pragma unroll
+    for (uint32_t q = 0; q < 8; q += 2) {
+      acc.w[0] = nrq_xor3(acc.w[0], d[q].x, d[q + 1].x); acc.w[1] = nrq_xor3(acc.w[1], d[q].y, d[q + 1].y);
+      acc.w[2] = nrq_xor3(acc.w[2], d[q].z, d[q + 1].z); acc.w[3] = nrq_xor3(acc.w[3], d[q].w, d[q + 1].w);
+    }
+    } else {
+      const uint32_t tb = (uint32_t)(uintptr_t)t4;
+#pragma unroll
+    for (uint32_t q = 0; q < 8; q++) {
+      const uint32_t a = t4_addr(tb, (q & 1u) ? odd : even, q >> 1) + (w * 8u + q) * 256u;
+      const uint4 v = *NRQ_LDSP(uint4, a);
+      acc.w[0] ^= v.x; acc.w[1] ^= v.y; acc.w[2] ^= v.z; acc.w[3] ^= v.w;
+      if (q == 3) NRQ_SCHED_FENCE();
+    }
+    }
+    NRQ_SCHED_FENCE();
+    return;
+  }
+  if constexpr (WB == 8 && G == 1) {
+    uint32_t odd = (bits >> 1) & 0x78787878u, even = (bits << 3) & 0x78787878u;
+    asm volatile("" : "+v"(odd), "+v"(even));
+    const uint32_t tbw = (uint32_t)(uintptr_t)t4 + w * 1024u;
+    uint2 d[8];
+#pragma unroll
+    for (uint32_t q = 0; q < 8; q++) d[q] = *NRQ_LDSP(uint2, t4_addr(tbw, (q & 1u) ? odd : even, q >> 1) + q * 128u);
+#pragma unroll
+    for (uint32_t q = 0; q < 8; q += 2) {
+      acc.w[0] = nrq_xor3(acc.w[0], d[q].x, d[q + 1].x); acc.w[1] = nrq_xor3(acc.w[1], d[q].y, d[q + 1].y);
+    }
+    NRQ_SCHED_FENCE();
+    return;
+  }
+  if constexpr (WB == 12 && G == 1) {
+    uint32_t odd = bits & 0xF0F0F0F0u, even = (bits << 4) & 0xF0F0F0F0u;
+    asm volatile("" : "+v"(odd), "+v"(even));
+    const uint32_t tbw = (uint32_t)(uintptr_t)t4 + w * 2048u;
+    uint4 d[8];
+#pragma unroll
+    for (uint32_t q = 0; q < 8; q++) d[q] = *NRQ_LDSP(uint4, t4_addr(tbw, (q & 1u) ? odd : even, q >> 1) + q * 256u);
+    uint32_t pad = 0;
+#pragma unroll
+    for (uint32_t q = 0; q < 8; q += 2) {
+      acc.w[0] = nrq_xor3(acc.w[0], d[q].x, d[q + 1].x); acc.w[1] = nrq_xor3(acc.w[1], d[q].y, d[q + 1].y);
+      acc.w[2] = nrq_xor3(acc.w[2], d[q].z, d[q + 1].z); pad = nrq_xor3(pad, d[q].w, d[q + 1].w);
+    }
+    asm volatile("" : : "v"(pad));
+    NRQ_SCHED_FENCE();
+    return;
+  }
+#endif
+#pragma unroll
+  for (uint32_t q = 0; q < 8; q++) {
+    const uint32_t nib = (bits >> (4u * q)) & 15u;
+    SV<WB> t = t4_get<WB, G>(t4, (w * 8u + q) * 16u + nib);
+    sv_xor<WB>(acc, t);
+    if (q == 3) NRQ_SCHED_FENCE();
+  }
+  NRQ_SCHED_FENCE();
+}
+template <int WB, int NW, int G = 1, bool FAST = true>
+SB_HD void t4_row(SV<WB> &acc, const uint8_t *t4, const uint32_t (&bitsw)[NW], uint32_t wpr) {
+#pragma unroll
+  for (uint32_t w = 0; w < (uint32_t)NW; w++) {
+    if (w >= wpr) break;
+    t4_word<WB, G, FAST>(acc, t4, w, bitsw[w]);
+  }
+}
 template <int WB, int NW, int G = 1, bool FAST = true>
 SB_HD void backsub_one(const StripCtx<WB, G> &c, const uint8_t *t4, uint32_t slot, const uint32_t (&bitsw)[NW],
                        uint32_t wpr) {
   SV<WB> acc = lds_get<WB, G>(c.slots(), slot);
-#pragma unroll
-  for (uint32_t w = 0; w < (uint32_t)NW; w++) {
-    if (w >= wpr) break;
-    const uint32_t bits = bitsw[w];
-#if defined(__HIP_DEVICE_COMPILE__)
-    if constexpr (WB == 16 && G == 1) {
-      uint32_t odd = bits & 0xF0F0F0F0u, even = (bits << 4) & 0xF0F0F0F0u;
-      asm volatile("" : "+v"(odd), "+v"(even));
-      if constexpr (FAST) {
-      const uint32_t tbw = (uint32_t)(uintptr_t)t4 + w * 2048u;
-      uint4 d[8];
-#pragma unroll
-      for (uint32_t q = 0; q < 8; q++) d[q] = *NRQ_LDSP(uint4, t4_addr(tbw, (q & 1u) ? odd : even, q >> 1) + q * 256u);
-#pragma unroll
-      for (uint32_t q = 0; q < 8; q += 2) {
-        acc.w[0] = nrq_xor3(acc.w[0], d[q].x, d[q + 1].x); acc.w[1] = nrq_xor3(acc.w[1], d[q].y, d[q + 1].y);
-        acc.w[2] = nrq_xor3(acc.w[2], d[q].z, d[q + 1].z); acc.w[3] = nrq_xor3(acc.w[3], d[q].w, d[q + 1].w);
-      }
-      } else {
-        const uint32_t tb = (uint32_t)(uintptr_t)t4;
-#pragma unroll
-      for (uint32_t q = 0; q < 8; q++) {
-        const uint32_t a = t4_addr(tb, (q & 1u) ? odd : even, q >> 1) + (w * 8u + q) * 256u;
-        const uint4 v = *NRQ_LDSP(uint4, a);
-        acc.w[0] ^= v.x; acc.w[1] ^= v.y; acc.w[2] ^= v.z; acc.w[3] ^= v.w;
-        if (q == 3) NRQ_SCHED_FENCE();
-      }
-      }
-      NRQ_SCHED_FENCE();
-      continue;
-    }
-    if constexpr (WB == 8 && G == 1) {
-      uint32_t odd = (bits >> 1) & 0x78787878u, even = (bits << 3) & 0x78787878u;
-      asm volatile("" : "+v"(odd), "+v"(even));
-      const uint32_t tbw = (uint32_t)(uintptr_t)t4 + w * 1024u;
-      uint2 d[8];
-#pragma unroll
-      for (uint32_t q = 0; q < 8; q++) d[q] = *NRQ_LDSP(uint2, t4_addr(tbw, (q & 1u) ? odd : even, q >> 1) + q * 128u);
-#pragma unroll
-      for (uint32_t q = 0; q < 8; q += 2) {
-        acc.w[0] = nrq_xor3(acc.w[0], d[q].x, d[q + 1].x); acc.w[1] = nrq_xor3(acc.w[1], d[q].y, d[q + 1].y);
-      }
-      NRQ_SCHED_FENCE();
-      continue;
-    }
-    if constexpr (WB == 12 && G == 1) {
-      uint32_t odd = bits & 0xF0F0F0F0u, even = (bits << 4) & 0xF0F0F0F0u;
-      asm volatile("" : "+v"(odd), "+v"(even));
-      const uint32_t tbw = (uint32_t)(uintptr_t)t4 + w * 2048u;
-      uint4 d[8];
-#pragma unroll
-      for (uint32_t q = 0; q < 8; q++) d[q] = *NRQ_LDSP(uint4, t4_addr(tbw, (q & 1u) ? odd : even, q >> 1) + q * 256u);
-      uint32_t pad = 0;
-#pragma unroll
-      for (uint32_t q = 0; q < 8; q += 2) {
-        acc.w[0] = nrq_xor3(acc.w[0], d[q].x, d[q + 1].x); acc.w[1] = nrq_xor3(acc.w[1], d[q].y, d[q + 1].y);
-        acc.w[2] = nrq_xor3(acc.w[2], d[q].z, d[q + 1].z); pad = nrq_xor3(pad, d[q].w, d[q + 1].w);
-      }
-      asm volatile("" : : "v"(pad));
-      NRQ_SCHED_FENCE();
-      continue;
-    }
-#endif
-#pragma unroll
-    for (uint32_t q = 0; q < 8; q++) {
-      const uint32_t nib = (bits >> (4u * q)) & 15u;
-      SV<WB> t = t4_get<WB, G>(t4, (w * 8u + q) * 16u + nib);
-      sv_xor<WB>(acc, t);
-      if (q == 3) NRQ_SCHED_FENCE();
-    }
-    NRQ_SCHED_FENCE();
-  }
+  t4_row<WB, NW, G, FAST>(acc, t4, bitsw, wpr);
   lds_put<WB, G>(c.slots(), slot, acc);
 }
 
@@ -1416,6 +1424,7 @@
 }
 
 template <int WB, int G = 1, bool FAST = true> SB_HD void ph_backsub(const StripCtx<WB, G> &c, uint32_t tid, uint32_t nt) {
+  if (nrq_job_out_view(c.job)) return;
   const uint32_t wpr = c.h->wpr;
   const bool need = c.job->inter == 0 && c.h->off_needslot != 0u;
   if (wpr <= 4) backsub_fixed<WB, 4, G, FAST>(c, need, tid, nt);
@@ -1482,25 +1491,25 @@
 SB_HD uint32_t store_slot(const uint32_t (&raw)[NRQ_STORE_TRIP / 2u], uint32_t k, uint32_t e, uint32_t end, uint32_t zero_at) {
   return e + k < end ? ((raw[k / 2u] >> (16u * (k & 1u))) & 0xFFFFu) + NRQ_SCRATCH : zero_at;
 }
-template <int WB, int G = 1, bool FAST = true> SB_HD void ph_store(const StripCtx<WB, G> &c, NRQ_GAS uint8_t *ostage, uint32_t tid, uint32_t nt) {
-  constexpr int STB = 8;
-  const NRQ_GAS uint16_t *colslot = c.template arr<uint16_t>(c.h->off_colslot);
-  const uint32_t L = c.h->L, ni = c.job->inter ? L : 0u;
-  for (uint32_t base = tid; base < ni; base += STB * nt) {
-    uint32_t sl[STB];
-#pragma unroll
-    for (int q = 0; q < STB; q++) {
-      uint32_t col = base + (uint32_t)q * nt;
-      sl[q] = col < L ? colslot[col] : 0u;
-    }
-#pragma unroll
-    for (int q = 0; q < STB; q++) {
-      uint32_t col = base + (uint32_t)q * nt;
-      if (col < L) g_put_stream<WB>(ostage + (size_t)col * (WB * G), WB, lds_get<WB, G>(c.slots(), sl[q]));
-    }
-  }
+template <int WB, int G, bool FAST> SB_HD void store_gen(const StripCtx<WB, G> &c, NRQ_GAS uint8_t *ostage, uint32_t ni, bool view, uint32_t tid, uint32_t nt) {
   const NRQ_GAS uint32_t *cptr = gptr<uint32_t>(c.job->out_cptr);
   const NRQ_GAS uint16_t *osl = gptr<uint16_t>(c.job->out_slots);
+  const uint32_t wpr = c.h->wpr, nlist = c.job->nout, opad = (nlist + 63u) & ~63u;
+  const NRQ_GAS uint32_t *wout = gptr<uint32_t>(c.job->plan + (view ? c.job->out_w : 0u));
+  const uint8_t *t4 = c.t4();
+  auto w_apply = [&](uint32_t q, SV<WB> &acc) {
+    if (!view) return;
+    for (uint32_t w0 = 0; w0 < wpr; w0 += 8u) {
+      uint32_t wb[8];
+#pragma unroll
+      for (uint32_t j = 0; j < 8u; j++) wb[j] = (w0 + j < wpr && q < nlist) ? wout[(size_t)(w0 + j) * opad + q] : 0u;
+#pragma unroll
+      for (uint32_t j = 0; j < 8u; j++) {
+        if (w0 + j >= wpr) break;
+        t4_word<WB, G, FAST>(acc, t4, w0 + j, wb[j]);
+      }
+    }
+  };
   if constexpr (FAST) {
   const uint32_t nout = c.job->nout;
   constexpr uint32_t CH = NRQ_STORE_CHUNK;
@@ -1531,6 +1540,7 @@
       }
       e += TR;
     }
+    w_apply(q, acc);
     if (q < nout) g_put_stream<WB>(ostage + (size_t)(ni + q) * (WB * G), WB, acc);
   }
   } else {
@@ -1552,9 +1562,29 @@
         if (sl[k] != NRQ_NOSLOT) sv_xor<WB>(acc, lds_get<WB, G>(c.slots(), sl[k]));
       e += CH;
     }
+    w_apply(q, acc);
     g_put_stream<WB>(ostage + (size_t)(ni + q) * (WB * G), WB, acc);
   }
   }
+}
+template <int WB, int G = 1, bool FAST = true> SB_HD void ph_store(const StripCtx<WB, G> &c, NRQ_GAS uint8_t *ostage, uint32_t tid, uint32_t nt) {
+  constexpr int STB = 8;
+  const NRQ_GAS uint16_t *colslot = c.template arr<uint16_t>(c.h->off_colslot);
+  const uint32_t L = c.h->L, ni = c.job->inter ? L : 0u;
+  for (uint32_t base = tid; base < ni; base += STB * nt) {
+    uint32_t sl[STB];
+#pragma unroll
+    for (int q = 0; q < STB; q++) {
+      uint32_t col = base + (uint32_t)q * nt;
+      sl[q] = col < L ? colslot[col] : 0u;
+    }
+#pragma unroll
+    for (int q = 0; q < STB; q++) {
+      uint32_t col = base + (uint32_t)q * nt;
+      if (col < L) g_put_stream<WB>(ostage + (size_t)col * (WB * G), WB, lds_get<WB, G>(c.slots(), sl[q]));
+    }
+  }
+  store_gen<WB, G, FAST>(c, ostage, ni, nrq_job_out_view(c.job), tid, nt);
 }
 template <int WB, int G = 1> SB_HD void ph_store_raw(const StripCtx<WB, G> &c, NRQ_GAS uint8_t *ostage, uint32_t tid, uint32_t nt) {
   const uint32_t M = c.h->M, u = c.h->u;
```

Result: faster. 1677 (median of 6 runs) (+2.0%).
